# DearCaat/MHIM-MIL

Hardware: AMD Instinct MI355X
Metric: patch-instances/sec through MHIM fwd+bwd, N=10k D=1024 (higher is better)
Workload: dtype f32; 1 GPU; c2: MHIM(ABMIL) train step, one bag N=10000 D=1024 per GPU per step (teacher fwd + select + student fwd + bwd + Adam + EMA); rotating_bags_per_gpu=8, matrix_core_form=bf16x3, parallelism=dp1, launch=hipGraph replay, one graph per resident bag

## Files before the change

include/mhimx.h:

```cpp
#ifndef MHIMX_H
#define MHIMX_H

#include <stdint.h>

#ifdef __cplusplus
extern "C" {
#endif

#define MHIMX_VERSION 620

enum { MHIMX_ACT_NONE = 0, MHIMX_ACT_RELU = 1, MHIMX_ACT_GELU = 2, MHIMX_ACT_TANH = 3 };

enum { MHIMX_PREC_F32 = 0, MHIMX_PREC_F16S = 1, MHIMX_PREC_BF16X3 = 2 };

const char* mhimx_last_error(void);
int mhimx_version(void);


typedef struct {
  const float* A; int64_t lda; const int64_t* rows;
  const float* B; int64_t ldb;
  float* C; int64_t ldc;
  int64_t M, N, K;
  const float* bias;
// ... 206 lines not shown
typedef struct { int64_t H, cell0, ncell, out0, out1; } mhimx_ppeg_band;
int64_t mhimx_ppeg_side(int64_t N, int64_t* wrapN);
int mhimx_ppeg_band_fwd(void* stream, const float* xb, const mhimx_ppeg_band* band, int64_t C, const float* wc, const float* bc, float* y);
int64_t mhimx_ppeg_band_bwd_ws_floats(int64_t n_out, int64_t C);
int mhimx_ppeg_band_bwd(void* stream, const float* dyb, const float* xb, const mhimx_ppeg_band* band, int64_t n_dw, int64_t C, const float* wc,
                        float* dx, float* dwc, float* dbc, float* ws);
int mhimx_scale_heads(void* stream, const float* v, int64_t ldv, const float* a, int64_t lda, int64_t dh, int64_t T, int64_t C, float* out);

int64_t mhimx_select_ws_bytes(int64_t N);
int mhimx_select_mask(void* stream, const float* score, int64_t N, int64_t k, int64_t n_sel, int32_t largest,
                      const int64_t* perm, const int64_t* other, int64_t n_other,
                      int64_t* mask_ids, int64_t* len_keep_dev, int64_t* topk_sorted ,
                      void* ws, int64_t ws_bytes);

int mhimx_select_rows(void* stream, const float* score, int64_t N, int64_t k, int64_t n_sel, int32_t largest,
                      uint64_t rand_seed, const uint64_t* tick, int64_t merge_R, int64_t* rows_out, int64_t* mask_ids,
                      void* ws, int64_t ws_bytes, int32_t merge_first );

int mhimx_select_rows_img(void* stream, const float* score, int64_t N, int64_t k, int64_t n_sel, int32_t largest, uint64_t rand_seed,
                          const uint64_t* tick, int64_t merge_R, int64_t* rows_out, int64_t* rows_img, int64_t img_merge_off, void* ws,
                          int64_t ws_bytes, int32_t merge_first);
int mhimx_vote_scores(void* stream, const float* attn, int64_t H, int64_t N, int64_t k, int32_t largest,
                      float* vote, void* ws, int64_t ws_bytes);

int mhimx_compose_ids(void* stream, const int64_t* a, const int64_t* b, int64_t* out, int64_t n);
int mhimx_random_perm(void* stream, int64_t n, uint64_t seed, const uint64_t* tick, const int64_t* src, int64_t* out);

typedef struct { int64_t row0, N, k, n_sel, merge_R, out0; uint64_t seed; } mhimx_select_bag;
int64_t mhimx_select_rows_many_ws_bytes(int32_t n_bags, const mhimx_select_bag* bags);
int mhimx_select_rows_many(void* stream, const float* score, int32_t n_bags, const mhimx_select_bag* bags, const uint64_t* tick,
                           int64_t* rows_out, void* ws, int64_t ws_bytes, int32_t merge_first);

typedef struct {
  int64_t E; int64_t k;
  int64_t heads; int64_t dim_head;
  const float* q_param;
  const float* ln_w; const float* ln_b;
  const float* wkv; const float* wq; const float* wo; const float* bo;
  const float* wkv_t; const float* wq_t; const float* wo_t;
  float mm;
  float drop_p; uint64_t drop_seed;
  int32_t prec;
  const uint64_t* drop_tick;
  const float* wkv_frag;
  const int64_t* x_rows;
  int32_t prepared;
  int64_t own_lo, own_n;
  float rep;
  int32_t rows_done;
} mhimx_merge;
int64_t mhimx_merge_ws_bytes(int64_t R, int64_t E, int64_t k, int64_t heads, int64_t dim_head);
int mhimx_merge_fwd(void* stream, const mhimx_merge* m, const float* X, int64_t R, float* z, float* q_new,
                    int32_t update_q, void* ws, int64_t ws_bytes);
typedef struct {
  float* d_ln_w; float* d_ln_b; float* d_wkv; float* d_wq; float* d_wo; float* d_bo;
  int32_t accumulate; int32_t splits;
  mhimx_reduce_list* defer;
} mhimx_merge_grad;
int64_t mhimx_merge_part_floats(void);
int mhimx_merge_fwd_part(void* stream, const mhimx_merge* m, const float* X, int64_t R, float* part, void* ws, int64_t ws_bytes);
int mhimx_merge_fwd_finish(void* stream, const mhimx_merge* m, const float* parts, int32_t W, int64_t R, float* z, float* q_new,
                           int32_t update_q, void* ws, int64_t ws_bytes);
int mhimx_merge_bwd(void* stream, const mhimx_merge* m, const float* X, int64_t R, const float* dz, float* dX,
                    const mhimx_merge_grad* g, void* ws, int64_t ws_bytes);
int mhimx_merge_bwd_park(const mhimx_merge* m, const float* X, int64_t R, const float* dz, float* dX, const mhimx_merge_grad* g, void* ws,
                         int64_t ws_bytes);

int mhimx_act_bwd(void* stream, float* dH, const float* H, const float* pre, int64_t M, int64_t E, int32_t act,
                  float drop_p, uint64_t drop_seed, const uint8_t* drop_mask, const int64_t* rows, float* colsum_out,
                  int32_t accumulate, void* ws, int64_t ws_bytes, const uint64_t* drop_tick);
int mhimx_mul_colsum(void* stream, float* dH, const float* dact, int64_t M, int64_t E, float* colsum_out, int32_t accumulate,
                     void* ws, int64_t ws_bytes, mhimx_reduce_list* defer );
int mhimx_rows_dpre(void* stream, const float* dH, const void* dact16, const int64_t* rows, int64_t L, int64_t E, float* dpre,
                    float* colsum_out, int32_t accumulate, void* ws, int64_t ws_bytes, mhimx_reduce_list* defer );
int64_t mhimx_wgrad_image_bytes(int64_t L, int64_t E);
int mhimx_rows_dpre_image(void* stream, const float* dH, const void* dact16, const int64_t* rows, int64_t L, int64_t E, void* img,
                          float* colsum_out, int32_t accumulate, void* ws, int64_t ws_bytes, mhimx_reduce_list* defer );
int mhimx_rows_dpre_image_c(void* stream, const float* dH_compact, const void* dact16, const int64_t* rows, int64_t L, int64_t E, void* img,
                            float* colsum_out, int32_t accumulate, void* ws, int64_t ws_bytes, mhimx_reduce_list* defer );
int mhimx_rows_dpre_image_k(void* stream, const float* dH, const void* dact16, const uint8_t* keep, int64_t N, int64_t E, void* img,
                            float* colsum_out, int32_t accumulate, void* ws, int64_t ws_bytes, mhimx_reduce_list* defer );
typedef struct {
  const void* img;
  const float* X; int64_t ldx; int64_t n_bag_rows;
  const int64_t* rows;
  int64_t L, E, D;
  float* C; int64_t ldc; int32_t accumulate;
  float* ws; int64_t ws_floats;
  mhimx_reduce_list* defer;
  int32_t ride_tail;
  const void* ximg;
} mhimx_bag_wgrad_args;
int64_t mhimx_wgrad_ws_floats(int64_t L, int64_t E, int64_t D);
int mhimx_bag_wgrad(void* stream, const mhimx_bag_wgrad_args* a);
int64_t mhimx_wgrad_multi_ws_floats(int64_t L, int64_t E, int64_t D, int32_t n_bags);
int mhimx_bag_wgrad_multi(void* stream, const mhimx_bag_wgrad_args* bags, int32_t n_bags);
int mhimx_shard_flags(void* stream, const int64_t* rows_all, int64_t R, int64_t Lk, int64_t lo, int64_t n, int64_t k_tokens,
                      int32_t tokens_live, uint8_t* excl);
int mhimx_shard_gather(void* stream, const float* H, int64_t E, const int64_t* rows, int64_t R, int64_t lo, int64_t n, float* out);
int mhimx_shard_scatter(void* stream, const float* dX, int64_t E, const int64_t* rows, int64_t R, int64_t lo, int64_t n, float* dH);
int mhimx_colsum(void* stream, const float* X, int64_t M, int64_t E, float* out, int32_t accumulate,
                 void* ws, int64_t ws_bytes);

int mhimx_head_fwd_bwd(void* stream, const float* z, const float* t, const float* wp, const float* bp,
                       const int64_t* label_dev, int64_t E, int64_t C, float temp_t, float main_alpha,
                       float aux_alpha, float inv_accum, float* logits, float* losses, float* g_z, float* d_wp,
// ... 320 lines not shown
```

mhim_mil_amd/_lib.py:

```python
from __future__ import annotations

import ctypes as C
import os

HERE = os.path.dirname(os.path.abspath(__file__))
LIB_PATH = os.path.join(HERE, os.environ.get("MHIMX_LIB_NAME", "libmhimx.so"))

c_f32p = C.c_void_p
c_i64p = C.c_void_p
c_u8p = C.c_void_p

ABI_VERSION = 620

ACT = {None: 0, "none": 0, "identity": 0, "relu": 1, "gelu": 2, "tanh": 3}
PREC = {"f32": 0, "f16s": 1, "bf16x3": 2}


def act_code(name, allowed):
    n = name.lower() if isinstance(name, str) else None
    return ACT[n] if n in allowed else 0


class GemmNT(C.Structure):
    _fields_ = [("A", c_f32p), ("lda", C.c_int64), ("rows", c_i64p),
# ... 54 lines not shown


class ParkedGemm(C.Structure):
    _fields_ = [("pending", C.c_int32), ("reserved", C.c_int32), ("blob", C.c_ubyte * 128)]


class ReduceListC(C.Structure):
    _fields_ = [("j", ReduceJob * REDUCE_MAX), ("n", C.c_int32), ("side", SideWork), ("parked", ParkedGemm), ("pre", SideWork)]


class GemmTN(C.Structure):
    _fields_ = [("A", c_f32p), ("lda", C.c_int64),
                ("B", c_f32p), ("ldb", C.c_int64), ("rows", c_i64p),
                ("C", c_f32p), ("ldc", C.c_int64),
                ("M", C.c_int64), ("K1", C.c_int64), ("K2", C.c_int64),
                ("splits", C.c_int32), ("ws", c_f32p),
                ("accumulate", C.c_int32), ("prec", C.c_int32), ("ws_floats", C.c_int64),
                ("defer", C.c_void_p)]


class Scorer(C.Structure):
    _fields_ = [("E", C.c_int64), ("A", C.c_int64), ("act", C.c_int32), ("gated", C.c_int32), ("prec", C.c_int32),
                ("wa", c_f32p), ("ba", c_f32p), ("wb", c_f32p), ("bb", c_f32p), ("wc", c_f32p), ("bc", c_f32p),
                ("wa_frag", c_f32p), ("gate_drop_p", C.c_float), ("gate_drop_seed", C.c_uint64)]


class PoolIO(C.Structure):
    _fields_ = [("T1", c_f32p), ("M1", C.c_int64), ("T2", c_f32p), ("M2", C.c_int64),
                ("s", c_f32p), ("stats", c_f32p), ("z", c_f32p), ("u_pre", c_f32p),
                ("wp", c_f32p), ("C", C.c_int64), ("cproj", c_f32p),
                ("ws", C.c_void_p), ("ws_bytes", C.c_int64), ("bp", c_f32p), ("pscore", c_f32p), ("rows1", c_i64p),
                ("excl", C.c_void_p), ("ride_jobs", C.c_void_p), ("n_ride_jobs", C.c_int32),
                ("phase", C.c_int32), ("tail_tokens", C.c_int32), ("ride_merge", C.c_void_p), ("ride_X", c_f32p), ("ride_R", C.c_int64),
                ("ride_ws", C.c_void_p), ("ride_ws_bytes", C.c_int64), ("rode_merge", C.c_int32), ("tail_wa_t", c_f32p), ("tail_row0", C.c_int64),
                ("no_backward", C.c_int32)]


class PoolGrad(C.Structure):
    _fields_ = [("g_z", c_f32p), ("dT1", c_f32p), ("dT2", c_f32p),
                ("d_wa", c_f32p), ("d_ba", c_f32p), ("d_wb", c_f32p), ("d_bb", c_f32p), ("d_wc", c_f32p),
                ("d_bc", c_f32p), ("wa_t", c_f32p), ("wb_t", c_f32p),
                ("accumulate", C.c_int32), ("splits", C.c_int32), ("defer", C.c_void_p), ("wa_t_frag", c_f32p),
                ("img", C.c_void_p), ("img_dact", C.c_void_p), ("img_part", c_f32p), ("img_rows", C.c_int64)]


class Merge(C.Structure):
    _fields_ = [("E", C.c_int64), ("k", C.c_int64), ("heads", C.c_int64), ("dim_head", C.c_int64),
                ("q_param", c_f32p), ("ln_w", c_f32p), ("ln_b", c_f32p),
                ("wkv", c_f32p), ("wq", c_f32p), ("wo", c_f32p), ("bo", c_f32p),
                ("wkv_t", c_f32p), ("wq_t", c_f32p), ("wo_t", c_f32p),
                ("mm", C.c_float), ("drop_p", C.c_float), ("drop_seed", C.c_uint64), ("prec", C.c_int32), ("drop_tick", C.c_void_p),
                ("wkv_frag", c_f32p), ("x_rows", c_i64p), ("prepared", C.c_int32), ("own_lo", C.c_int64), ("own_n", C.c_int64),
                ("rep", C.c_float), ("rows_done", C.c_int32)]


class MergeGrad(C.Structure):
    _fields_ = [("d_ln_w", c_f32p), ("d_ln_b", c_f32p), ("d_wkv", c_f32p), ("d_wq", c_f32p), ("d_wo", c_f32p),
                ("d_bo", c_f32p), ("accumulate", C.c_int32), ("splits", C.c_int32), ("defer", C.c_void_p)]


_P = C.c_void_p
_I64 = C.c_int64
_I32 = C.c_int32
_F = C.c_float
_U64 = C.c_uint64


class Nys(C.Structure):
    _fields_ = [("q", C.c_void_p), ("k", C.c_void_p), ("v", C.c_void_p), ("ld", C.c_int64), ("T", C.c_int64),
                ("ql", C.c_void_p), ("kl", C.c_void_p), ("ldl", C.c_int64), ("scale", C.c_float),
                ("ws", C.c_void_p), ("ws_floats", C.c_int64)]


class BmmStep(C.Structure):
    _fields_ = [("A", C.c_void_p), ("B", C.c_void_p), ("C", C.c_void_p), ("PN", C.c_void_p), ("PT", C.c_void_p),
                ("PN2", C.c_void_p), ("PT2", C.c_void_p), ("D", C.c_void_p), ("D2", C.c_void_p), ("alpha", C.c_float), ("ident", C.c_float),
                ("alpha2", C.c_float), ("ident2", C.c_float), ("dscale", C.c_float), ("d2scale", C.c_float), ("kind", C.c_int32)]


class OptimArgs(C.Structure):
    _fields_ = [("p", C.c_void_p), ("g", C.c_void_p), ("m", C.c_void_p), ("v", C.c_void_p), ("teacher", C.c_void_p),
                ("n_train", C.c_int64), ("n_all", C.c_int64), ("step", C.c_int64), ("step_dev", C.c_void_p),
                ("lr", C.c_float), ("lr_table", C.c_void_p), ("lr_len", C.c_int64),
                ("beta1", C.c_float), ("beta2", C.c_float), ("eps", C.c_float), ("weight_decay", C.c_float), ("grad_scale", C.c_float),
                ("ema_mm", C.c_float), ("mm_table", C.c_void_p), ("mm_len", C.c_int64), ("zero_grad", C.c_int32),
                ("g_extra", C.c_void_p), ("n_extra", C.c_int64), ("extra_pitch", C.c_int64), ("clip_norm", C.c_float),
                ("ws", C.c_void_p), ("ws_floats", C.c_int64), ("fold", C.c_void_p), ("extra_lo", C.c_int64), ("extra_only", C.c_int32)]


class StepParams(C.Structure):
    _fields_ = [(n, C.c_void_p) for n in ("w1", "b1", "wa", "wc", "wp", "bp", "q", "ln_w", "ln_b", "wkv", "wq", "wo", "bo")]


class StepGrads(C.Structure):
    _fields_ = [(n, C.c_void_p) for n in ("w1", "b1", "wa", "wc", "wp", "bp", "ln_w", "ln_b", "wkv", "wq", "wo", "bo")]


class StepCfg(C.Structure):
    _fields_ = [("D", C.c_int64), ("E", C.c_int64), ("A", C.c_int64), ("C", C.c_int64), ("k", C.c_int64),
                ("act", C.c_int32), ("da_act", C.c_int32), ("attn2score", C.c_int32),
                ("drop_p_teacher", C.c_float), ("drop_p_student", C.c_float), ("merge_drop_p", C.c_float), ("merge_mm", C.c_float),
                ("temp_t", C.c_float), ("main_alpha", C.c_float), ("aux_alpha", C.c_float),
                ("student", StepParams), ("teacher", StepParams), ("grad", StepGrads),
                ("p", C.c_void_p), ("g", C.c_void_p), ("m", C.c_void_p), ("v", C.c_void_p), ("p_teacher", C.c_void_p),
                ("n_train", C.c_int64), ("n_all", C.c_int64),
                ("lr", C.c_float), ("beta1", C.c_float), ("beta2", C.c_float), ("eps", C.c_float), ("weight_decay", C.c_float), ("ema_mm", C.c_float),
# ... 128 lines not shown
                                        "H_teacher", "H_student", "dact", "score", "rows_all", "tokens")] + [
        ("row0", C.c_int64 * DSMIL_MHIM_WINDOW_MAX), ("tok0", C.c_int64 * DSMIL_MHIM_WINDOW_MAX)]


RAGGED_WINDOW_MAX = 32
RAGGED_WINDOW_MAX_ROWS = 524288


class RaggedWindowBag(C.Structure):
    _fields_ = [("X", c_f32p), ("ldx", C.c_int64), ("N", C.c_int64), ("label_dev", C.c_void_p), ("cnt", StepCounts), ("seeds", StepSeeds)]


class RaggedWindowLayout(C.Structure):
    _fields_ = [(n, C.c_int64) for n in ("total", "rows", "logits", "losses", "score", "rows_all", "H_teacher", "H_student", "dact", "dpre",
                                        "z_teacher", "z_student")] + [("row0", C.c_int64 * RAGGED_WINDOW_MAX)]


class SurvSpec(C.Structure):
    _fields_ = [("alpha", C.c_float), ("eps", C.c_float), ("censor_dev", C.c_void_p * INFER_MAX), ("risk", C.c_void_p)]


SYMBOLS = {
    "mhimx_last_error": (C.c_char_p, []),
    "mhimx_version": (C.c_int, []),
    "mhimx_gemm_nt": (C.c_int, [_P, C.POINTER(GemmNT)]),
    "mhimx_pool_finalize": (C.c_int, [_P, _P, _P, _P, _I64, _I64, _P, _P, _P, _P, _P, _I64, _I64, _P]),
    "mhimx_proj_score_parts": (_I64, [_I64]),
    "mhimx_proj_score_xch_floats": (_I64, [_I64]),
    "mhimx_bag_project": (C.c_int, [_P, C.POINTER(BagProject)]),
    "mhimx_bag_project_multi": (C.c_int, [_P, _P, _I32]),
    "mhimx_gemm_nn": (C.c_int, [_P, C.POINTER(GemmNT), _F, _I32, _P]),
    "mhimx_prep_batch": (C.c_int, [_P, C.POINTER(PrepJob), _I32]),
    "mhimx_pair_planes": (C.c_int, [_P, _P, _I64, _I64, _I64, _P]),
    "mhimx_lse_merge": (C.c_int, [_P, _P, _I64, _I64, _P, _P]),
    "mhimx_gemm_batched": (C.c_int, [_P, _I32, C.POINTER(GemmNT), _I32, _I64, _I64, _I64, _F, _I32, _P]),
    "mhimx_gemm_tn": (C.c_int, [_P, C.POINTER(GemmTN)]),
    "mhimx_transpose": (C.c_int, [_P, _P, _P, _I64, _I64]),
    "mhimx_abmil_pool_ws_bytes": (_I64, [_I64, _I64, _I64, _I32]),
    "mhimx_abmil_pool_fwd": (C.c_int, [_P, C.POINTER(Scorer), C.POINTER(PoolIO)]),
    "mhimx_abmil_pool_bwd": (C.c_int, [_P, C.POINTER(Scorer), C.POINTER(PoolIO), C.POINTER(PoolGrad)]),
    "mhimx_softmax_from_stats": (C.c_int, [_P, _P, _P, _P, _I64]),
    "mhimx_pseudo_score": (C.c_int, [_P, _P, _P, _P, _P, _P, _P, _I64, _I64]),
    "mhimx_select_ws_bytes": (_I64, [_I64]),
    "mhimx_select_mask": (C.c_int, [_P, _P, _I64, _I64, _I64, _I32, _P, _P, _I64, _P, _P, _P, _P, _I64]),
    "mhimx_select_rows": (C.c_int, [_P, _P, _I64, _I64, _I64, _I32, _U64, _P, _I64, _P, _P, _P, _I64, _I32]),
    "mhimx_select_rows_img": (C.c_int, [_P, _P, _I64, _I64, _I64, _I32, _U64, _P, _I64, _P, _P, _I64, _P, _I64, _I32]),
    "mhimx_vote_scores": (C.c_int, [_P, _P, _I64, _I64, _I64, _I32, _P, _P, _I64]),
    "mhimx_compose_ids": (C.c_int, [_P, _P, _P, _P, _I64]),
    "mhimx_random_perm": (C.c_int, [_P, _I64, _U64, _P, _P, _P]),
    "mhimx_select_rows_many_ws_bytes": (_I64, [_I32, _P]),
    "mhimx_select_rows_many": (C.c_int, [_P, _P, _I32, _P, _P, _P, _P, _I64, _I32]),
    "mhimx_merge_ws_bytes": (_I64, [_I64, _I64, _I64, _I64, _I64]),
    "mhimx_merge_fwd": (C.c_int, [_P, C.POINTER(Merge), _P, _I64, _P, _P, _I32, _P, _I64]),
    "mhimx_merge_part_floats": (_I64, []),
    "mhimx_merge_fwd_part": (C.c_int, [_P, C.POINTER(Merge), _P, _I64, _P, _P, _I64]),
    "mhimx_merge_fwd_finish": (C.c_int, [_P, C.POINTER(Merge), _P, _I32, _I64, _P, _P, _I32, _P, _I64]),
    "mhimx_merge_bwd": (C.c_int, [_P, C.POINTER(Merge), _P, _I64, _P, _P, C.POINTER(MergeGrad), _P, _I64]),
    "mhimx_merge_bwd_park": (C.c_int, [C.POINTER(Merge), _P, _I64, _P, _P, C.POINTER(MergeGrad), _P, _I64]),
    "mhimx_act_bwd": (C.c_int, [_P, _P, _P, _P, _I64, _I64, _I32, _F, _U64, _P, _P, _P, _I32, _P, _I64, _P]),
    "mhimx_softmax_cols": (C.c_int, [_P, _P, _P, _I64, _I64, _F]),
    "mhimx_softmax_cols_bwd": (C.c_int, [_P, _P, _P, _P, _I64, _I64, _F]),
    "mhimx_colmax": (C.c_int, [_P, _P, _I64, _I64, _P, _P]),
    "mhimx_rowmax": (C.c_int, [_P, _P, _I64, _I64, _P]),
    "mhimx_dsmil_head": (C.c_int, [_P, _P, _P, _P, _P, _P, _I64, _I64, _F, _F, _F, _F, _P, _P, _P, _P, _P]),
    "mhimx_mul_colsum": (C.c_int, [_P, _P, _P, _I64, _I64, _P, _I32, _P, _I64, _P]),
    "mhimx_rows_dpre": (C.c_int, [_P, _P, _P, _P, _I64, _I64, _P, _P, _I32, _P, _I64, _P]),
    "mhimx_bmm_affine": (C.c_int, [_P, _I32, _P, _I32, _I64, _I64, _I64, C.c_float, C.c_float]),
    "mhimx_bmm_affine2": (C.c_int, [_P, _I32, _P, _I32, _I64, _I64, _I64, C.c_float, C.c_float, _P, C.c_float, C.c_float]),
    "mhimx_bmm_affine_pair": (C.c_int, [_P, _I32, C.POINTER(GemmNT), _F, _F, _I32, C.POINTER(GemmNT), _F, _F, _I32, _I64]),
    "mhimx_shard_flags": (C.c_int, [_P, _P, _I64, _I64, _I64, _I64, _I64, _I32, _P]),
    "mhimx_shard_gather": (C.c_int, [_P, _P, _I64, _P, _I64, _I64, _I64, _P]),
    "mhimx_shard_scatter": (C.c_int, [_P, _P, _I64, _P, _I64, _I64, _I64, _P]),
    "mhimx_rows_dpre_image": (C.c_int, [_P, _P, _P, _P, _I64, _I64, _P, _P, _I32, _P, _I64, _P]),
    "mhimx_rows_dpre_image_c": (C.c_int, [_P, _P, _P, _P, _I64, _I64, _P, _P, _I32, _P, _I64, _P]),
    "mhimx_rows_dpre_image_k": (C.c_int, [_P, _P, _P, _P, _I64, _I64, _P, _P, _I32, _P, _I64, _P]),
    "mhimx_wgrad_image_bytes": (_I64, [_I64, _I64]),
    "mhimx_wgrad_ws_floats": (_I64, [_I64, _I64, _I64]),
    "mhimx_bag_wgrad": (C.c_int, [_P, _P]),
    "mhimx_bag_wgrad_multi": (C.c_int, [_P, _P, _I32]),
    "mhimx_wgrad_multi_ws_floats": (C.c_int64, [_I64, _I64, _I64, _I32]),
    "mhimx_reduce_flush": (C.c_int, [_P, _P]),
    "mhimx_cls_metrics_ws_bytes": (C.c_int64, [_I64, _I64, _I64]),
    "mhimx_cls_metrics": (C.c_int, [_P, _P, _I64, _P, _I64, _I64, _I32, _P, _I64, _P, _P, _I64]),
    "mhimx_surv_nll": (C.c_int, [_P, _P, _I64, _P, _P, _I64, _I64, _F, _F, _F, _P, _P, _P]),
    "mhimx_cindex_ws_bytes": (C.c_int64, [_I64, _I64]),
    "mhimx_cindex": (C.c_int, [_P, _P, _P, _P, _I64, _P, _I64, _F, _P, _P, _I64]),
    "mhimx_colsum": (C.c_int, [_P, _P, _I64, _I64, _P, _I32, _P, _I64]),
    "mhimx_head_fwd_bwd": (C.c_int, [_P, _P, _P, _P, _P, _P, _I64, _I64, _F, _F, _F, _F, _P, _P, _P, _P, _P, _I32, _P, _P]),
    "mhimx_head_surv_fwd_bwd": (C.c_int, [_P, _P, _P, _P, _P, _P, _P, _I64, _I64, _F, _F, _F, _F, _F, _F, _P, _P, _P, _P, _P, _P, _I32]),
    "mhimx_adam_ema": (C.c_int, [_P, _P, _P, _P, _P, _P, _I64, _I64, _I64, _F, _F, _F, _F, _F, _F, _F, _I32, _P, _P, _I64]),
    "mhimx_bmm_chain": (C.c_int, [_P, C.POINTER(BmmStep), _I32, _I32, _P]),
    "mhimx_optim_step": (C.c_int, [_P, C.POINTER(OptimArgs)]),
    "mhimx_stream_copy": (C.c_int, [_P, _P, _P, _I64]),
    "mhimx_tick": (C.c_int, [_P, _P]),
    "mhimx_layernorm_fwd": (C.c_int, [_P, _P, _I64, _I64, _P, _P, _P, _P, _P]),
    "mhimx_layernorm_bwd": (C.c_int, [_P, _P, _P, _I64, _I64, _P, _P, _P, _P, _P, _P, _I32, _P]),
    "mhimx_layernorm_bwd_res": (C.c_int, [_P, _P, _P, _I64, _I64, _P, _P, _P, _P, _P, _P, _P, _I32, _P]),
    "mhimx_dropout_apply": (C.c_int, [_P, _P, _P, _I64, _I64, _F, _U64, _P]),
    "mhimx_dropout_apply_proj": (C.c_int, [_P, _P, _P, _I64, _I64, _F, _U64, _P]),
    "mhimx_softmax_rows": (C.c_int, [_P, _P, _P, _I64, _I64, _F]),
    "mhimx_softmax_rows_bwd": (C.c_int, [_P, _P, _P, _P, _I64, _I64, _F]),
    "mhimx_landmark_mean": (C.c_int, [_P, _P, _I64, _I64, _I64, _I64, _P]),
    "mhimx_landmark_mean_bwd": (C.c_int, [_P, _P, _I64, _I64, _I64, _P, _I64, _I32]),
    "mhimx_affine_ident": (C.c_int, [_P, _P, _P, _I64, _I64, _F, _F]),
    "mhimx_axpby": (C.c_int, [_P, _P, _P, _I64, _F, _F]),
    "mhimx_pinv_init": (C.c_int, [_P, _P, _I64, _I64, _P, _P, _P]),
# ... 92 lines not shown
```

mhim_mil_amd/csrc/common.hpp:

```cpp
#pragma once
#include <hip/hip_runtime.h>
#include <stdint.h>
#include <stdio.h>
#include <string>
#include <type_traits>

#include "../../include/mhimx.h"

namespace mhimx {

void set_error(const std::string& s);
int fail(int code, const char* fmt, ...);
const std::string& last_error();

#define MHIMX_CHECK_ARG(cond, ...)                      \
  do {                                                  \
    if (!(cond)) return ::mhimx::fail(-1, __VA_ARGS__); \
  } while (0)

#define MHIMX_HIP(expr)                                                                      \
  do {                                                                                       \
    hipError_t _e = (expr);                                                                  \
    if (_e != hipSuccess) return ::mhimx::fail((int)_e, "%s: %s", #expr, hipGetErrorString(_e)); \
  } while (0)
// ... 38 lines not shown
}
inline bool reduce_slabs_as_parts(int64_t splits, int64_t K1, int64_t K2, int64_t ldo) { return splits >= 32 && ldo == K2 && K1 * K2 <= 16384; }
inline mhimx_reduce_job reduce_job_slabs(const float* ws, int64_t splits, int64_t K1, int64_t K2, int64_t ldo, float* out, int accumulate) {
  if (reduce_slabs_as_parts(splits, K1, K2, ldo)) return reduce_job_parts(ws, splits, K1 * K2, K1 * K2, out, accumulate);
  mhimx_reduce_job j = {};
  j.kind = 1; j.accumulate = accumulate; j.parts = ws; j.out = out; j.G = splits; j.K1 = K1; j.K2 = K2; j.ldo = ldo;
  return j;
}

int reduce_parts_now(hipStream_t st, const float* part, int64_t G, int64_t W, int64_t ld, float* out, int accumulate);
int reduce_slabs_now(hipStream_t st, const float* ws, float* C, int64_t K1, int64_t K2, int64_t ldc, int splits, int accumulate,
                     int batch = 1, int64_t sC = 0);

inline mhimx_optim_args optim_args_of(const mhimx_step_cfg& c, int64_t host_step, bool with_teacher) {
  mhimx_optim_args o = {};
  o.p = c.p; o.g = c.g; o.m = c.m; o.v = c.v; o.n_train = c.n_train; o.n_all = c.n_all; o.step = host_step; o.step_dev = c.opt_step;
  o.lr = c.lr; o.lr_table = c.lr_table; o.lr_len = c.lr_len; o.beta1 = c.beta1; o.beta2 = c.beta2; o.eps = c.eps; o.weight_decay = c.weight_decay;
  o.grad_scale = 1.f; o.zero_grad = 1;
  if (with_teacher) { o.teacher = c.p_teacher; o.ema_mm = c.ema_mm; o.mm_table = c.mm_table; o.mm_len = c.mm_len; }
  return o;
}

inline int prep_counters(const mhimx_step_cfg& c, mhimx_prep_job* j) {
  int n = 0;
  j[n++] = mhimx_prep_job{3, nullptr, reinterpret_cast<float*>(c.tick), 1, 1};
  if (c.opt_step) j[n++] = mhimx_prep_job{3, nullptr, reinterpret_cast<float*>(c.opt_step), 1, 1};
  return n;
}

struct Arena {
  char* base;
  int64_t cap, off;
  Arena(void* p, int64_t bytes) : base((char*)p), cap(bytes), off(0) {}
  template <typename T>
  T* take(int64_t n) {
    int64_t b = align_up(n * (int64_t)sizeof(T), 256);
    T* r = (T*)(base + off);
    off += b;
    return r;
  }
  bool ok() const { return off <= cap && (base != nullptr || off == 0); }
};

constexpr int BAG_BATCH_MAX = MHIMX_WINDOW_MAX;
struct BagBatch {
  int32_t n, pad;
  uint64_t lo[3], span[3];
  int64_t stride[3];
  uint64_t dsel[BAG_BATCH_MAX], dmca[BAG_BATCH_MAX];
  uint64_t tab_key, tab[BAG_BATCH_MAX];
};
const BagBatch& cur_batch();
void set_batch(const BagBatch* b);
inline dim3 bgrid(unsigned x, unsigned y = 1) { return dim3(x, y, cur_batch().n > 0 ? (unsigned)cur_batch().n : 1u); }

#define MHIMX_DEV __device__ __forceinline__

template <typename T>
MHIMX_DEV T* bag_ptr(T* p, const BagBatch& bb) {
  const unsigned bag = blockIdx.z;
  if (bag == 0) return p;
  const uint64_t a = reinterpret_cast<uint64_t>(p);
#pragma unroll
  for (int r = 0; r < 3; ++r)
    if (a - bb.lo[r] < bb.span[r]) return reinterpret_cast<T*>(a + (uint64_t)bag * (uint64_t)bb.stride[r]);
  if (a == bb.tab_key) return reinterpret_cast<T*>(bb.tab[bag]);
  return p;
}
#define MHIMX_BAG(p) p = ::mhimx::bag_ptr(p, bb)
MHIMX_DEV uint64_t bag_sel_seed(uint64_t s, const BagBatch& bb) { return blockIdx.z ? s + bb.dsel[blockIdx.z] : s; }
MHIMX_DEV uint64_t bag_mca_seed(uint64_t s, const BagBatch& bb) { return blockIdx.z ? s + bb.dmca[blockIdx.z] : s; }

MHIMX_DEV float erf_fast(float x) {
  const float ax = fabsf(x);
  const float t = __frcp_rn(fmaf(0.3275911f, ax, 1.f));
  float p = fmaf(1.061405429f, t, -1.453152027f);
  p = fmaf(p, t, 1.421413741f);
  p = fmaf(p, t, -0.284496736f);
  p = fmaf(p, t, 0.254829592f);
  const float r = 1.f - p * t * __expf(-ax * ax);
  return copysignf(r, x);
}

MHIMX_DEV float tanh_fast(float x) {
  const float t = __expf(-2.f * fabsf(x));
  return copysignf((1.f - t) * __frcp_rn(1.f + t), x);
}

MHIMX_DEV float act_fwd(float x, int act) {
  switch (act) {
    case MHIMX_ACT_RELU: return x > 0.f ? x : 0.f;
    case MHIMX_ACT_GELU: return 0.5f * x * (1.f + erf_fast(x * 0.70710678118654752440f));
    case MHIMX_ACT_TANH: return tanh_fast(x);
    default: return x;
  }
}

MHIMX_DEV float act_grad(float x, float y, int act) {
  switch (act) {
    case MHIMX_ACT_RELU: return y > 0.f ? 1.f : 0.f;
    case MHIMX_ACT_GELU: {
      const float phi = 0.39894228040143267794f * __expf(-0.5f * x * x);
      return 0.5f * (1.f + erf_fast(x * 0.70710678118654752440f)) + x * phi;
    }
    case MHIMX_ACT_TANH: return 1.f - y * y;
    default: return 1.f;
// ... 114 lines not shown
```

mhim_mil_amd/csrc/dsmil_mhim.hip:

```cpp
#include <math.h>
#include <string.h>

#include "infer_tab.hpp"

namespace mhimx {

bool merge2_ok(const mhimx_merge* m, int64_t R);
int64_t merge2_ws_bytes(int64_t R, int64_t k);

namespace {

constexpr int DM_Q = 128, DM_MAXC = 16, DM_ROWS = RG_ROWS, DM_T = 256;
constexpr int DM_MAX = MHIMX_DSMIL_MHIM_WINDOW_MAX;
constexpr int DM_GATHER_Y = 64;
static_assert(DM_MAX == MHIMX_INFER_MAX, "the by-value bag table is the inference call's");

typedef _Float16 dm_h4 __attribute__((ext_vector_type(4)));

struct DmCnt {
  int64_t tok0[DM_MAX], mrg0[DM_MAX];
  int32_t len_keep[DM_MAX], Lk[DM_MAX], tslot[DM_MAX];
};
struct DmLabels { const int64_t* p[DM_MAX]; };

__global__ __launch_bounds__(DM_T) void dm_gather_kernel(InferTab tab, DmCnt cn, const float* __restrict__ Hs, const int64_t* __restrict__ rows_all,
                                                         int k, float* __restrict__ T, float* __restrict__ Xm, int32_t* __restrict__ pos) {
  const int bag = blockIdx.x;
  int64_t N = tab.N[0], orow0 = tab.row0[0], tok0 = cn.tok0[0], mrg0 = cn.mrg0[0];
  int len_keep = cn.len_keep[0], Lk = cn.Lk[0], tslot = cn.tslot[0];
  RG_PICK(N, tab.N, bag) RG_PICK(orow0, tab.row0, bag) RG_PICK(tok0, cn.tok0, bag) RG_PICK(mrg0, cn.mrg0, bag)
  RG_PICK(len_keep, cn.len_keep, bag) RG_PICK(Lk, cn.Lk, bag) RG_PICK(tslot, cn.tslot, bag)
  const int tid = threadIdx.x, lane = tid & 63, wave = tid >> 6;
  const int64_t* rows = rows_all + orow0;
  const f32x4 z4 = f32x4{0.f, 0.f, 0.f, 0.f};
  for (int j = blockIdx.y * (DM_T / 64) + wave; j < len_keep; j += (DM_T / 64) * gridDim.y) {
    const int64_t r = rows[j];
    const bool ok = r >= 0 && r < N;
    const f32x4* src = reinterpret_cast<const f32x4*>(Hs + (orow0 + (ok ? r : 0)) * IE);
    f32x4* dst = reinterpret_cast<f32x4*>(j < Lk ? T + (tok0 + j) * IE : Xm + (mrg0 + (j - Lk)) * IE);
    f32x4 v0 = src[lane], v1 = src[lane + 64];
    if (!ok) { v0 = z4; v1 = z4; }
    dst[lane] = v0;
    dst[lane + 64] = v1;
    if (ok && lane == 0) pos[orow0 + r] = j;
  }
  if (blockIdx.y == 0) {
    const int first = Lk + k;
    f32x4* dst = reinterpret_cast<f32x4*>(T + (tok0 + first) * IE);
    for (int f = tid; f < (tslot - first) * (IE / 4); f += DM_T) dst[f] = z4;
  }
}

MHIMX_DEV float dm_blk_max(float v, float* red) {
  const int lane = threadIdx.x & 63, wave = threadIdx.x >> 6;
  v = wave_max(v);
  if (lane == 0) red[wave] = v;
  __syncthreads();
  float r = red[0];
#pragma unroll
  for (int w = 1; w < 8; ++w) r = fmaxf(r, red[w]);
  __syncthreads();
// ... 142 lines not shown
}

__global__ __launch_bounds__(DM_T) void dm_scatter_kernel(InferTab tab, DmCnt cn, const int64_t* __restrict__ rows_all, const int32_t* __restrict__ pos,
                                                          const float* __restrict__ dT, const float* __restrict__ dXm,
                                                          const _Float16* __restrict__ dact, float* __restrict__ dpre, float* __restrict__ part) {
  __shared__ f32x4 half[IE / 4];
  __shared__ int64_t srow[DM_ROWS];
  const int tile = blockIdx.x, tid = threadIdx.x;
  const int64_t r0 = (int64_t)tile * DM_ROWS;
  RG_FIND_BAG(r0, row0)
  int64_t N = tab.N[0], orow0 = tab.row0[0], tok0 = cn.tok0[0], mrg0 = cn.mrg0[0];
  int len_keep = cn.len_keep[0], Lk = cn.Lk[0];
  RG_PICK(N, tab.N, bag) RG_PICK(orow0, tab.row0, bag) RG_PICK(tok0, cn.tok0, bag) RG_PICK(mrg0, cn.mrg0, bag)
  RG_PICK(len_keep, cn.len_keep, bag) RG_PICK(Lk, cn.Lk, bag)
  if (tid < DM_ROWS) {
    const int64_t rin = r0 - orow0 + tid;
    int64_t s = -1;
    if (rin < N) {
      const int p = pos[r0 + tid];
      if (p >= 0 && p < len_keep && rows_all[orow0 + p] == rin) s = p < Lk ? tok0 + p : -2 - (mrg0 + (p - Lk));
    }
    srow[tid] = s;
  }
  __syncthreads();
  const int c4 = tid & 127, par = tid >> 7;
  f32x4 sum = f32x4{0.f, 0.f, 0.f, 0.f};
#pragma unroll 4
  for (int i = 0; i < DM_ROWS / 2; ++i) {
    const int r = 2 * i + par;
    const int64_t s = srow[r];
    f32x4 d = f32x4{0.f, 0.f, 0.f, 0.f};
    if (s != -1) {
      const float* src = s >= 0 ? dT + s * IE : dXm + (-2 - s) * IE;
      const f32x4 g = reinterpret_cast<const f32x4*>(src)[c4];
      const dm_h4 a = *(reinterpret_cast<const dm_h4*>(dact + (r0 + r) * IE) + c4);
#pragma unroll
      for (int q = 0; q < 4; ++q) d[q] = g[q] * (float)a[q];
    }
    *(reinterpret_cast<f32x4*>(dpre + (r0 + r) * IE) + c4) = d;
#pragma unroll
    for (int q = 0; q < 4; ++q) sum[q] += d[q];
  }
  if (par == 1) half[c4] = sum;
  __syncthreads();
  if (par == 0) {
    const f32x4 o = half[c4];
#pragma unroll
    for (int q = 0; q < 4; ++q) sum[q] += o[q];
    *(reinterpret_cast<f32x4*>(part + (int64_t)tile * IE) + c4) = sum;
  }
}

struct DmLay {
  int64_t w1p_t, w1p_s, vp_t, q0f_t, q2f_t, vp, vtp, q0f, q2f, q2tf, q0tf, wo_t;
  int64_t logits, losses, logits_bag, logits_ins, B, crit, B_t, lb_t, lg_t, li_t, crit_t, qmax_t, qmax, stats, gli, dB, delta, dqmax, dwfcc_part,
      dbfcc_part, dwi_part, dbi_part;
  int64_t H_t, H_s, dact, V_t, Q_t, cls_t, score, rows_all, pos, db1_part, pmax_t, parg_t, pm_t, pl_t, pB_t, slab_1;
  int64_t T, V, dhv, Q, cls, da, U1, dPQ, dP1, pmax, parg, pm, pl, pB, dbv_part, dbq0_part, dbq2_part, dqm_part, slab_v, slab_q0, slab_q2;
  int64_t Xm, dXm, merge_ws[DM_MAX], merge_ws_bytes[DM_MAX], sel_ws, sel_ws_bytes, sel_perm, sel_ids, sel_rows, sel_lk;
  int64_t total, rows, trows, mrows;
  int32_t steps, tsteps, s1, s1_per, sv, sv_per, sq0, sq0_per, sq2, sq2_per;
};

mhimx_merge dm_merge_params(const mhimx_dsmil_mhim_cfg& c) {
  mhimx_merge m = {};
  m.E = c.base.E; m.k = c.k; m.heads = 8; m.dim_head = 64;
  m.q_param = c.q; m.ln_w = c.merge.ln_w; m.ln_b = c.merge.ln_b; m.wkv = c.merge.wkv; m.wq = c.merge.wq; m.wo = c.merge.wo; m.bo = c.merge.bo;
  m.mm = c.merge_mm; m.prec = MHIMX_PREC_BF16X3; m.drop_tick = c.base.tick; m.rep = 1.f; m.drop_p = c.merge_drop_p;
  return m;
}

bool dm_params_ok(const mhimx_dsmil_params& p) {
  return p.w1 && p.b1 && p.wi && p.bi && p.wq0 && p.bq0 && p.wq2 && p.bq2 && p.wv && p.bv && p.wfcc && p.bfcc;
}
bool dm_params_aligned(const mhimx_dsmil_params& p) {
  return aligned16(p.w1) && aligned16(p.b1) && aligned16(p.wi) && aligned16(p.wq0) && aligned16(p.wq2) && aligned16(p.wv) && aligned16(p.bv);
}

int check_dm(const mhimx_dsmil_mhim_cfg* cfg, int32_t n_bags, const mhimx_ragged_window_bag* bags, int32_t xdt = MHIMX_X_F32) {
  const char* who = "dsmil_mhim_window";
  if (int r = rg_check_xdt(who, xdt)) return r;
  MHIMX_CHECK_ARG(cfg && bags, "dsmil_mhim_window: null configuration / bag list");
  MHIMX_CHECK_ARG(n_bags >= 1 && n_bags <= DM_MAX, "dsmil_mhim_window: 1..%d bags per window (got %d)", DM_MAX, n_bags);
  const mhimx_dsmil_train_cfg* c = &cfg->base;
  MHIMX_CHECK_ARG(c->E == IE && c->C >= 1 && c->C <= DM_MAXC && c->D > 0 && c->D % 256 == 0 && c->D <= (1 << 20),
                  "dsmil_mhim_window: shapes outside the ragged MHIM(DSMIL) window (E = 512, q width 128, 1 <= C <= %d, D %% 256 == 0, D <= 2^20)", DM_MAXC);
  MHIMX_CHECK_ARG(cfg->k >= 1 && 8 * cfg->k <= 48, "dsmil_mhim_window: merge_k outside 1..6 (8 k <= 48)");
  MHIMX_CHECK_ARG(c->act >= MHIMX_ACT_NONE && c->act <= MHIMX_ACT_TANH, "dsmil_mhim_window: unknown activation");
  MHIMX_CHECK_ARG(c->drop_p >= 0.f && c->drop_p < 1.f && cfg->drop_p_teacher >= 0.f && cfg->drop_p_teacher < 1.f && cfg->merge_drop_p >= 0.f &&
                      cfg->merge_drop_p < 1.f,
                  "dsmil_mhim_window: dropout probability outside [0,1)");
  MHIMX_CHECK_ARG(cfg->temp_t > 0.f, "dsmil_mhim_window: the distillation temperature must be positive");
  MHIMX_CHECK_ARG(dm_params_ok(c->param), "dsmil_mhim_window: null student parameter");
  MHIMX_CHECK_ARG(dm_params_ok(cfg->teacher), "dsmil_mhim_window: null teacher parameter");
  MHIMX_CHECK_ARG(dm_params_aligned(c->param) && dm_params_aligned(cfg->teacher),
                  "dsmil_mhim_window: the feature, i_classifier, q and v weights of both models must be 16-byte aligned");
  const mhimx_dsmil_grads& g = c->grad;
  MHIMX_CHECK_ARG(g.w1 && g.b1 && g.wi && g.bi && g.wq0 && g.bq0 && g.wq2 && g.bq2 && g.wv && g.bv && g.wfcc && g.bfcc,
                  "dsmil_mhim_window: null gradient view");
  const mhimx_dsmil_merge_params& m = cfg->merge;
  MHIMX_CHECK_ARG(m.ln_w && m.ln_b && m.wkv && m.wq && m.wo && m.bo && cfg->q, "dsmil_mhim_window: null Merge parameter / global queries");
  MHIMX_CHECK_ARG(aligned16(m.ln_w) && aligned16(m.ln_b) && aligned16(m.wkv) && aligned16(m.wq) && aligned16(m.wo) && aligned16(cfg->q) &&
                      (!cfg->q_out || aligned16(cfg->q_out)),
                  "dsmil_mhim_window: the Merge weights and the global queries must be 16-byte aligned");
  const mhimx_dsmil_merge_grads& mg = cfg->merge_grad;
  MHIMX_CHECK_ARG(mg.ln_w && mg.ln_b && mg.wkv && mg.wq && mg.wo && mg.bo, "dsmil_mhim_window: null Merge gradient view");
  MHIMX_CHECK_ARG(c->tick, "dsmil_mhim_window: the device dropout / draw counter (tick) is required");
// ... 11 lines not shown
    MHIMX_CHECK_ARG(merge2_ok(&mw, n.R), "dsmil_mhim_window: bag %d: the Merge entry points' projection-free form does not take R = %lld", b,
                    (long long)n.R);
    rows += align_up(q.N, DM_ROWS);
    MHIMX_CHECK_ARG(rows <= MHIMX_DSMIL_MHIM_WINDOW_MAX_ROWS, "dsmil_mhim_window: bag %d: %lld rows in the window's bag space up to this bag, at most %d", b,
                    (long long)rows, MHIMX_DSMIL_MHIM_WINDOW_MAX_ROWS);
  }
  return 0;
}

void dm_layout(const mhimx_dsmil_mhim_cfg* cfg, int32_t n_bags, const mhimx_ragged_window_bag* bags, DmLay* w, InferTab* tab, InferTab* tab2, DmCnt* cn,
               int64_t* row0_out, int64_t* tok0_out) {
  const int64_t E = cfg->base.E, D = cfg->base.D, C = cfg->base.C, k = cfg->k, n = n_bags;
  RgCount cnt, cnt2;
  int64_t mrows = 0, sel_b = 0, perm_n = 0, ids_n = 0, rows_n = 0;
  for (int b = 0; b < n_bags; ++b) {
    const mhimx_ragged_window_bag& q = bags[b];
    const int64_t M = q.cnt.Lk + k, tslot = align_up(M, DM_ROWS);
    if (row0_out) row0_out[b] = cnt.rows;
    if (tok0_out) tok0_out[b] = cnt2.rows;
    if (cn) {
      cn->tok0[b] = cnt2.rows; cn->mrg0[b] = mrows; cn->len_keep[b] = (int32_t)q.cnt.len_keep; cn->Lk[b] = (int32_t)q.cnt.Lk;
      cn->tslot[b] = (int32_t)tslot;
    }
    rg_tab_add(tab, cnt, b, q.X, q.ldx, q.N, align_up(q.N, DM_ROWS));
    rg_tab_add(tab2, cnt2, b, nullptr, IE, M, tslot);
    mrows += q.cnt.R;
    auto up = [](int64_t& a, int64_t v) { if (v > a) a = v; };
    up(sel_b, mhimx_select_ws_bytes(q.N));
    if (q.N > 16384) { up(perm_n, q.cnt.k_top); up(ids_n, q.N); up(rows_n, q.cnt.len_keep); }
  }
  rg_tab_close(tab, cnt, n_bags);
  rg_tab_close(tab2, cnt2, n_bags);
  const int64_t rows = cnt.rows, parts = cnt.parts, trows = cnt2.rows, tparts = cnt2.parts;
  w->rows = rows; w->trows = trows; w->mrows = mrows;
  w->steps = (int32_t)(rows / DM_ROWS);
  w->tsteps = (int32_t)(trows / DM_ROWS);
  const int s1_room = pw_split_k(w->steps, 8, 8, &w->s1, &w->s1_per);
  const int sv_room = pw_split_k(w->tsteps, 16, 4, &w->sv, &w->sv_per);
  const int sq0_room = pw_split_k(w->tsteps, 64, 4, &w->sq0, &w->sq0_per);
  const int sq2_room = pw_split_k(w->tsteps, 64, 2, &w->sq2, &w->sq2_per);
  Arena ar(nullptr, 0);
  w->w1p_t = ar.off; ar.take<float>(E * D);
  w->w1p_s = ar.off; ar.take<float>(E * D);
  w->vp_t = ar.off; ar.take<float>(E * E);
  w->q0f_t = ar.off; ar.take<float>(DM_Q * E);
  w->q2f_t = ar.off; ar.take<float>(DM_Q * DM_Q);
  w->vp = ar.off; ar.take<float>(E * E);
  w->vtp = ar.off; ar.take<float>(E * E);
  w->q0f = ar.off; ar.take<float>(DM_Q * E);
  w->q2f = ar.off; ar.take<float>(DM_Q * DM_Q);
  w->q2tf = ar.off; ar.take<float>(DM_Q * DM_Q);
  w->q0tf = ar.off; ar.take<float>(DM_Q * E);
  w->wo_t = ar.off; ar.take<float>(512 * E);
  w->logits = ar.off; ar.take<float>(n * C);
  w->losses = ar.off; ar.take<float>(n * 3);
  w->logits_bag = ar.off; ar.take<float>(n * C);
  w->logits_ins = ar.off; ar.take<float>(n * C);
  w->B = ar.off; ar.take<float>(n * C * E);
  w->crit = ar.off; ar.take<int64_t>(n * C);
  w->B_t = ar.off; ar.take<float>(n * C * E);
  w->lb_t = ar.off; ar.take<float>(n * C);
  w->lg_t = ar.off; ar.take<float>(n * C);
  w->li_t = ar.off; ar.take<float>(n * C);
  w->crit_t = ar.off; ar.take<int64_t>(n * C);
  w->qmax_t = ar.off; ar.take<float>(n * DM_MAXC * DM_Q);
  w->qmax = ar.off; ar.take<float>(n * DM_MAXC * DM_Q);
  w->stats = ar.off; ar.take<float>(n * DM_MAXC * 2);
  w->gli = ar.off; ar.take<float>(n * DM_MAXC);
  w->dB = ar.off; ar.take<float>(n * DM_MAXC * E);
  w->delta = ar.off; ar.take<float>(n * DM_MAXC);
  w->dqmax = ar.off; ar.take<float>(n * DM_MAXC * DM_Q);
  w->dwfcc_part = ar.off; ar.take<float>(n * C * C * E);
  w->dbfcc_part = ar.off; ar.take<float>(n * C);
  w->dwi_part = ar.off; ar.take<float>(n * C * E);
  w->dbi_part = ar.off; ar.take<float>(n * C);
  w->H_t = ar.off; ar.take<float>(rows * E);
  w->H_s = ar.off; ar.take<float>(rows * E);
  w->dact = ar.off; ar.take<_Float16>(rows * E);
  w->V_t = ar.off; ar.take<float>(rows * E);
  w->Q_t = ar.off; ar.take<float>(rows * DM_Q);
  w->cls_t = ar.off; ar.take<float>(rows * DM_MAXC);
  w->score = ar.off; ar.take<float>(rows);
  w->rows_all = ar.off; ar.take<int64_t>(rows);
  w->pos = ar.off; ar.take<int32_t>(rows);
  w->db1_part = ar.off; ar.take<float>((int64_t)w->steps * E);
  w->pmax_t = ar.off; ar.take<float>(parts * DM_MAXC);
  w->parg_t = ar.off; ar.take<int32_t>(parts * DM_MAXC);
  w->pm_t = ar.off; ar.take<float>(parts * DM_MAXC);
  w->pl_t = ar.off; ar.take<float>(parts * DM_MAXC);
  w->pB_t = ar.off; ar.take<float>(parts * C * E);
  w->slab_1 = ar.off; ar.take<float>((int64_t)s1_room * E * D);
  w->T = ar.off; ar.take<float>(trows * E);
  w->V = ar.off; ar.take<float>(trows * E);
  w->dhv = ar.off; ar.take<float>(trows * E);
  w->Q = ar.off; ar.take<float>(trows * DM_Q);
  w->cls = ar.off; ar.take<float>(trows * DM_MAXC);
  w->da = ar.off; ar.take<float>(trows * DM_MAXC);
  w->U1 = ar.off; ar.take<float>(trows * DM_Q);
  w->dPQ = ar.off; ar.take<float>(trows * DM_Q);
  w->dP1 = ar.off; ar.take<float>(trows * DM_Q);
  w->pmax = ar.off; ar.take<float>(tparts * DM_MAXC);
  w->parg = ar.off; ar.take<int32_t>(tparts * DM_MAXC);
  w->pm = ar.off; ar.take<float>(tparts * DM_MAXC);
  w->pl = ar.off; ar.take<float>(tparts * DM_MAXC);
  w->pB = ar.off; ar.take<float>(tparts * C * E);
  w->dbv_part = ar.off; ar.take<float>((int64_t)w->tsteps * E);
  w->dbq0_part = ar.off; ar.take<float>((int64_t)w->tsteps * DM_Q);
  w->dbq2_part = ar.off; ar.take<float>((int64_t)w->tsteps * DM_Q);
  w->dqm_part = ar.off; ar.take<float>((int64_t)w->tsteps * DM_MAXC * DM_Q);
  w->slab_v = ar.off; ar.take<float>((int64_t)sv_room * E * E);
  w->slab_q0 = ar.off; ar.take<float>((int64_t)sq0_room * DM_Q * E);
  w->slab_q2 = ar.off; ar.take<float>((int64_t)sq2_room * DM_Q * DM_Q);
  w->Xm = ar.off; ar.take<float>(mrows * E);
  w->dXm = ar.off; ar.take<float>(mrows * E);
  for (int b = 0; b < n_bags; ++b) {
    w->merge_ws_bytes[b] = merge2_ws_bytes(bags[b].cnt.R, k);
    w->merge_ws[b] = ar.off; ar.take<char>(w->merge_ws_bytes[b]);
  }
  w->sel_ws_bytes = sel_b; w->sel_ws = ar.off; ar.take<char>(sel_b);
  w->sel_perm = ar.off; ar.take<int64_t>(perm_n);
  w->sel_ids = ar.off; ar.take<int64_t>(ids_n);
  w->sel_rows = ar.off; ar.take<int64_t>(rows_n);
  w->sel_lk = ar.off; ar.take<int64_t>(1);
  w->total = ar.off;
}

}

}

using namespace mhimx;

extern "C" int mhimx_dsmil_mhim_window_layout_of(const mhimx_dsmil_mhim_cfg* cfg, int32_t n_bags, const mhimx_ragged_window_bag* bags,
                                                 mhimx_dsmil_mhim_window_layout* out) {
  MHIMX_CHECK_ARG(out, "dsmil_mhim_window_layout: null output");
  if (int r = check_dm(cfg, n_bags, bags)) return r;
  DmLay w;
  memset(out, 0, sizeof(*out));
  dm_layout(cfg, n_bags, bags, &w, nullptr, nullptr, nullptr, out->row0, out->tok0);
  out->total = w.total; out->rows = w.rows; out->tok_rows = w.trows; out->logits = w.logits; out->losses = w.losses; out->logits_bag = w.logits_bag;
  out->logits_ins = w.logits_ins; out->B = w.B; out->crit = w.crit; out->B_teacher = w.B_t; out->H_teacher = w.H_t; out->H_student = w.H_s;
  out->dact = w.dact; out->score = w.score; out->rows_all = w.rows_all; out->tokens = w.T;
  return 0;
}

extern "C" int64_t mhimx_dsmil_mhim_window_ws_bytes(const mhimx_dsmil_mhim_cfg* cfg, int32_t n_bags, const mhimx_ragged_window_bag* bags) {
  if (int r = check_dm(cfg, n_bags, bags)) return r;
  DmLay w;
  dm_layout(cfg, n_bags, bags, &w, nullptr, nullptr, nullptr, nullptr, nullptr);
  return w.total;
}

extern "C" int mhimx_dsmil_mhim_window_run(void* stream, const mhimx_dsmil_mhim_cfg* cfg, int32_t n_bags, const mhimx_ragged_window_bag* bags,
                                           int64_t host_step, void* ws, int64_t ws_bytes, int32_t update, int32_t x_dtype) {
  if (int r = check_dm(cfg, n_bags, bags, x_dtype)) return r;
  for (int b = 0; b < n_bags; ++b) {
    MHIMX_CHECK_ARG(bags[b].X && aligned16(bags[b].X), "dsmil_mhim_window: bag %d: null or unaligned rows", b);
    MHIMX_CHECK_ARG(bags[b].label_dev, "dsmil_mhim_window: bag %d: null label", b);
  }
  const mhimx_dsmil_train_cfg& c = cfg->base;
  MHIMX_CHECK_ARG(!update || (c.p && c.g && c.m && c.v && c.n_train > 0 && c.n_all >= c.n_train), "dsmil_mhim_window: update needs the flat optimiser buffers");
  DmLay w;
  InferTab tab = {}, tab2 = {};
  DmCnt cn = {};
  dm_layout(cfg, n_bags, bags, &w, &tab, &tab2, &cn, nullptr, nullptr);
  tab.pad = x_dtype;
  tab2.pad = MHIMX_X_F32;
  if (int r = rg_check_ws("dsmil_mhim_window", ws, ws_bytes, w.total)) return r;
  const mhimx_dsmil_params &P = c.param, &Tp = cfg->teacher;
  hipStream_t st = (hipStream_t)stream;
  char* base = static_cast<char*>(ws);
  auto F = [&](int64_t off) { return reinterpret_cast<float*>(base + off); };
  const int D = (int)c.D, C = (int)c.C;
  const int64_t k = cfg->k;
  float *H_t = F(w.H_t), *H_s = F(w.H_s), *V_t = F(w.V_t), *Q_t = F(w.Q_t), *score = F(w.score);
  float *T = F(w.T), *V = F(w.V), *dhv = F(w.dhv), *Q = F(w.Q), *Xm = F(w.Xm), *dXm = F(w.dXm);
  float* dpre = V_t;
  _Float16* dact = reinterpret_cast<_Float16*>(base + w.dact);
  int64_t* rows_space = reinterpret_cast<int64_t*>(base + w.rows_all);
  int32_t* pos = reinterpret_cast<int32_t*>(base + w.pos);
  int64_t* crit = reinterpret_cast<int64_t*>(base + w.crit);
  const uint64_t* tick = c.tick;
  float* q_dst = cfg->q_out ? cfg->q_out : cfg->q;

  mhimx_merge mw_prep = dm_merge_params(*cfg);
  {
    mhimx_prep_job jobs[24];
    int n = 0;
    jobs[n++] = mhimx_prep_job{3, nullptr, reinterpret_cast<float*>(c.tick), 1, 1};
    if (c.opt_step) jobs[n++] = mhimx_prep_job{3, nullptr, reinterpret_cast<float*>(c.opt_step), 1, 1};
    jobs[n++] = mhimx_prep_job{1, Tp.w1, F(w.w1p_t), c.E, c.D};
    jobs[n++] = mhimx_prep_job{1, P.w1, F(w.w1p_s), c.E, c.D};
    jobs[n++] = mhimx_prep_job{1, Tp.wv, F(w.vp_t), c.E, c.E};
    jobs[n++] = mhimx_prep_job{4, Tp.wq0, F(w.q0f_t), DM_Q, c.E};
    jobs[n++] = mhimx_prep_job{4, Tp.wq2, F(w.q2f_t), DM_Q, DM_Q};
    jobs[n++] = mhimx_prep_job{1, P.wv, F(w.vp), c.E, c.E};
    jobs[n++] = mhimx_prep_job{7, P.wv, F(w.vtp), c.E, c.E};
    jobs[n++] = mhimx_prep_job{4, P.wq0, F(w.q0f), DM_Q, c.E};
    jobs[n++] = mhimx_prep_job{4, P.wq2, F(w.q2f), DM_Q, DM_Q};
    jobs[n++] = mhimx_prep_job{5, P.wq2, F(w.q2tf), DM_Q, DM_Q};
    jobs[n++] = mhimx_prep_job{5, P.wq0, F(w.q0tf), DM_Q, c.E};
    jobs[n++] = mhimx_prep_job{0, cfg->merge.wo, F(w.wo_t), c.E, 512};
    if (cfg->q_out) jobs[n++] = mhimx_prep_job{2, cfg->q, cfg->q_out, 1, k * c.E};
    for (int b = 0; b < n_bags && b < 8; ++b)
      jobs[n++] = mhimx_prep_job{6, reinterpret_cast<const float*>(&mw_prep), reinterpret_cast<float*>(base + w.merge_ws[b]), bags[b].cnt.R, w.merge_ws_bytes[b]};
    if (int r = mhimx_prep_batch(stream, jobs, n)) return r;
  }
  {
    PureWinDrop dr = {};
    dr.tick = tick; dr.dact = dact;
    for (int b = 0; b < n_bags; ++b) dr.seed[b] = bags[b].seeds.drop_teacher;
    dr.drop_p = cfg->drop_p_teacher;
    if (int r = pure_window_project(st, tab, dr, D, F(w.w1p_t), Tp.b1, c.act, H_t)) return r;
    for (int b = 0; b < n_bags; ++b) dr.seed[b] = bags[b].seeds.drop_student;
    dr.drop_p = c.drop_p;
    if (int r = pure_window_project(st, tab, dr, D, F(w.w1p_s), P.b1, c.act, H_s)) return r;
  }
  InferTab tabv = tab;
  for (int b = 0; b < n_bags; ++b) { tabv.X[b] = H_t + tab.row0[b] * IE; tabv.ldx[b] = IE; }
  tabv.pad = MHIMX_X_F32;
  if (int r = infer_project(st, tabv, IE, F(w.vp_t), Tp.bv, MHIMX_ACT_RELU, V_t)) return r;
  if (int r = dsmil_rows_crit_pool(st, tab, H_t, V_t, F(w.q0f_t), Tp.bq0, F(w.q2f_t), Tp.bq2, Tp.wi, Tp.bi, C, Q_t, F(w.cls_t), F(w.pmax_t),
                                   reinterpret_cast<int32_t*>(base + w.parg_t), F(w.qmax_t), F(w.li_t), reinterpret_cast<int64_t*>(base + w.crit_t),
                                   F(w.pm_t), F(w.pl_t), F(w.pB_t), cfg->cls_attn ? score : nullptr))
    return r;
  if (int r = dsmil_finalize(st, tab, F(w.pm_t), F(w.pl_t), F(w.pB_t), Q_t, F(w.qmax_t), Tp.wfcc, Tp.bfcc, C, F(w.li_t), F(w.lb_t), F(w.lg_t), F(w.B_t),
                             cfg->cls_attn ? nullptr : score))
    return r;
  {
    mhimx_select_bag sb[DM_MAX];
    for (int b = 0; b < n_bags; ++b) {
      const mhimx_step_counts& n = bags[b].cnt;
      sb[b] = mhimx_select_bag{tab.row0[b], bags[b].N, n.k_top, n.n_sel, n.R, tab.row0[b], bags[b].seeds.select};
    }
    SelLargeWs lw;
    lw.perm = reinterpret_cast<int64_t*>(base + w.sel_perm); lw.ids = reinterpret_cast<int64_t*>(base + w.sel_ids);
    lw.rows = reinterpret_cast<int64_t*>(base + w.sel_rows); lw.lk = reinterpret_cast<int64_t*>(base + w.sel_lk);
    lw.sel_ws = base + w.sel_ws; lw.sel_ws_bytes = w.sel_ws_bytes;
    if (int r = select_bags_check("dsmil_mhim_window", n_bags, sb)) return r;
    if (int r = select_rows_many_launch(st, score, n_bags, sb, tick, rows_space, lw, 0)) return r;
  }
  hipLaunchKernelGGL(dm_gather_kernel, dim3((unsigned)n_bags, DM_GATHER_Y), dim3(DM_T), 0, st, tab, cn, H_s, rows_space, (int)k, T, Xm, pos);
  MHIMX_LAUNCH_CHECK();

  for (int b = 0; b < n_bags; ++b) {
    if (b >= 8 && b % 8 == 0) {
      mhimx_prep_job jobs[8];
      int n = 0;
      for (int q = b; q < n_bags && q < b + 8; ++q)
        jobs[n++] = mhimx_prep_job{6, reinterpret_cast<const float*>(&mw_prep), reinterpret_cast<float*>(base + w.merge_ws[q]), bags[q].cnt.R, w.merge_ws_bytes[q]};
      if (int r = mhimx_prep_batch(stream, jobs, n)) return r;
    }
    mhimx_merge mw = mw_prep;
    mw.drop_seed = bags[b].seeds.mca; mw.prepared = 1;
    if (int r = mhimx_merge_fwd(stream, &mw, Xm + cn.mrg0[b] * IE, bags[b].cnt.R, T + (cn.tok0[b] + cn.Lk[b]) * IE, nullptr, 0, base + w.merge_ws[b],
                                w.merge_ws_bytes[b]))
      return r;
  }

  InferTab tabt = tab2;
  for (int b = 0; b < n_bags; ++b) tabt.X[b] = T + tab2.row0[b] * IE;
  if (int r = infer_project(st, tabt, IE, F(w.vp), P.bv, MHIMX_ACT_RELU, V)) return r;
  if (int r = dsmil_rows_crit_pool(st, tab2, T, V, F(w.q0f), P.bq0, F(w.q2f), P.bq2, P.wi, P.bi, C, Q, F(w.cls), F(w.pmax),
                                   reinterpret_cast<int32_t*>(base + w.parg), F(w.qmax), F(w.logits_ins), crit, F(w.pm), F(w.pl), F(w.pB)))
    return r;
  {
    DmLabels lab = {};
    for (int b = 0; b < n_bags; ++b) lab.p[b] = bags[b].label_dev;
    const float* Bt = cfg->aux_alpha != 0.f ? F(w.B_t) : nullptr;
    hipLaunchKernelGGL(dm_head_kernel, dim3((unsigned)n_bags), dim3(RG_FIN_T), 0, st, tab2, lab, F(w.pm), F(w.pl), F(w.pB), T, P.wfcc, P.bfcc, F(w.logits_ins),
                       crit, Bt, C, cfg->temp_t, c.main_alpha, cfg->aux_alpha, 1.f / (float)n_bags, F(w.logits_bag), F(w.logits), F(w.losses), F(w.B),
                       F(w.stats), F(w.gli), F(w.dB), F(w.delta), F(w.dwfcc_part), F(w.dbfcc_part), F(w.dwi_part), F(w.dbi_part));
    MHIMX_LAUNCH_CHECK();
  }
  if (int r = dw_rows1(st, tab2, w.tsteps, V, Q, F(w.qmax), F(w.stats), F(w.dB), F(w.delta), C, F(w.da), F(w.dbv_part), F(w.dqm_part))) return r;
  for (int b = 0; b < n_bags; ++b) tabt.X[b] = V + tab2.row0[b] * IE;
  if (int r = infer_project(st, tabt, IE, F(w.vtp), nullptr, MHIMX_ACT_NONE, dhv)) return r;
  if (int r = dw_dqmax(st, tab2, F(w.dqm_part), F(w.dqmax))) return r;
  if (int r = dw_rows2_plain(st, tab2, w.tsteps, T, Q, F(w.da), F(w.qmax), F(w.dqmax), crit, F(w.gli), P.wi, F(w.q0f), P.bq0, F(w.q2tf), F(w.q0tf), C, dhv,
                             F(w.U1), F(w.dPQ), F(w.dP1), F(w.dbq0_part), F(w.dbq2_part)))
    return r;
  if (int r = pw_wgrad_rows(st, tab2, V, IE, IE, T, IE, IE, w.tsteps, w.sv, w.sv_per, F(w.slab_v))) return r;
  if (int r = pw_wgrad_rows(st, tab2, F(w.dPQ), DM_Q, DM_Q, F(w.U1), DM_Q, DM_Q, w.tsteps, w.sq2, w.sq2_per, F(w.slab_q2))) return r;
  if (int r = pw_wgrad_rows(st, tab2, F(w.dP1), DM_Q, DM_Q, T, IE, IE, w.tsteps, w.sq0, w.sq0_per, F(w.slab_q0))) return r;

  for (int b = 0; b < n_bags; ++b) {
    mhimx_merge mwb = mw_prep;
    mwb.drop_seed = bags[b].seeds.mca; mwb.wo_t = F(w.wo_t); mwb.prepared = 0;
    mhimx_reduce_list lst;
    memset(&lst, 0, sizeof(lst));
    mhimx_merge_grad mg = {};
    const mhimx_dsmil_merge_grads& G_ = cfg->merge_grad;
    mg.d_ln_w = G_.ln_w; mg.d_ln_b = G_.ln_b; mg.d_wkv = G_.wkv; mg.d_wq = G_.wq; mg.d_wo = G_.wo; mg.d_bo = G_.bo;
    mg.accumulate = b > 0 ? 1 : 0; mg.splits = 8; mg.defer = &lst;
    if (int r = mhimx_merge_bwd(stream, &mwb, Xm + cn.mrg0[b] * IE, bags[b].cnt.R, dhv + (cn.tok0[b] + cn.Lk[b]) * IE, dXm + cn.mrg0[b] * IE, &mg,
                                base + w.merge_ws[b], w.merge_ws_bytes[b]))
      return r;
    if (int r = mhimx_reduce_flush(stream, &lst)) return r;
  }

  hipLaunchKernelGGL(dm_scatter_kernel, dim3((unsigned)w.steps), dim3(DM_T), 0, st, tab, cn, rows_space, pos, dhv, dXm, dact, dpre, F(w.db1_part));
  MHIMX_LAUNCH_CHECK();
  if (int r = pw_wgrad_bagx(st, tab, dpre, D, w.steps, w.s1, w.s1_per, F(w.slab_1))) return r;
// ... 27 lines not shown
```

mhim_mil_amd/csrc/errors.hip:

```cpp
#include <stdarg.h>

#include "common.hpp"

namespace mhimx {
static thread_local std::string g_err;
void set_error(const std::string& s) { g_err = s; }
int fail(int code, const char* fmt, ...) {
  char buf[512];
  va_list ap;
  va_start(ap, fmt);
  vsnprintf(buf, sizeof(buf), fmt, ap);
  va_end(ap);
  g_err = buf;
  return code;
}
const std::string& last_error() { return g_err; }

static thread_local BagBatch g_batch = {};
const BagBatch& cur_batch() { return g_batch; }
void set_batch(const BagBatch* b) {
  if (b) g_batch = *b;
  else g_batch = BagBatch{};
}
}

extern "C" const char* mhimx_last_error(void) { return mhimx::last_error().c_str(); }
extern "C" int mhimx_version(void) { return MHIMX_VERSION; }
```

mhim_mil_amd/csrc/gemm_dma.hip:

```cpp
#include <string.h>

#include "common.hpp"
#include "mca2_rows.hpp"
#include "prep_jobs.hpp"

namespace mhimx {

typedef float f32x16 __attribute__((ext_vector_type(16)));
typedef float f4 __attribute__((ext_vector_type(4)));
typedef _Float16 h8 __attribute__((ext_vector_type(8)));
typedef __bf16 b8 __attribute__((ext_vector_type(8)));
typedef __attribute__((address_space(1))) const void* gptr_t;
typedef __attribute__((address_space(3))) void* lptr_t;

constexpr int DBM = 128, DBN = 128, DBK = 32, DTHREADS = 256;
constexpr int TILE_BYTES = 128 * DBK * 4;
constexpr int STAGE_BYTES = 2 * TILE_BYTES;
#ifndef MHIMX_NT_STAGES
#define MHIMX_NT_STAGES 2
#endif
constexpr int NSTAGE = MHIMX_NT_STAGES;
constexpr int NT_LDS_BYTES = NSTAGE * STAGE_BYTES > DBM * (DBN + 8) * 4 ? NSTAGE * STAGE_BYTES : DBM * (DBN + 8) * 4;
#define LDS_READ8(x, a, off)                                                                                         \
  asm volatile("ds_read_b128 %0, %8\n\tds_read_b128 %1, %9\n\tds_read_b128 %2, %10\n\tds_read_b128 %3, %11\n\t"       \
// ... 421 lines not shown
        const int64_t i = i0 + wm * 64 + mt * 32 + (e & 3) + 8 * (e >> 2) + 4 * rh;
        float v = acc[mt][nt][e];
        float* p = out + i * ldo + j;
        if (accum) v += *p;
        *p = v;
      }
    }
}


__global__ void pair_planes_kernel(const float* __restrict__ x, int64_t ldx, int64_t M, int64_t K8, float* __restrict__ out) {
  const int64_t n = M * K8;
  for (int64_t i = (int64_t)blockIdx.x * blockDim.x + threadIdx.x; i < n; i += (int64_t)gridDim.x * blockDim.x) {
    const int64_t m = i / K8, g8 = i % K8;
    const f4 a = *reinterpret_cast<const f4*>(x + m * ldx + g8 * 8);
    const f4 b = *reinterpret_cast<const f4*>(x + m * ldx + g8 * 8 + 4);
    b8 hi, lo;
    Frag<MHIMX_PREC_BF16X3>::split2(a, b, hi, lo);
    f4* o = reinterpret_cast<f4*>(out + (m * K8 + g8) * 8);
    o[0] = __builtin_bit_cast(f4, hi);
    o[1] = __builtin_bit_cast(f4, lo);
  }
}
int pair_planes(hipStream_t st, const float* x, int64_t ldx, int64_t M, int64_t K, float* out) {
  MHIMX_CHECK_ARG(x && out && M > 0 && K > 0 && K % 8 == 0 && ldx % 4 == 0 && aligned16(x) && aligned16(out),
                  "pair_planes: K must be a multiple of 8, rows 16-byte aligned");
  const int64_t n = M * (K / 8);
  int64_t blocks = cdiv(n, 256);
  if (blocks > 8192) blocks = 8192;
  hipLaunchKernelGGL(pair_planes_kernel, dim3((unsigned)blocks), dim3(256), 0, st, x, ldx, M, K / 8, out);
  MHIMX_LAUNCH_CHECK();
  return 0;
}

__global__ __launch_bounds__(256) void prep_batch_kernel(PrepJobs pj) {
  __shared__ __attribute__((aligned(16))) float lds[PREP_LDS_FLOATS];
  prep_job_block(pj, (int)blockIdx.x, lds);
}
int merge2_prep_args(const mhimx_merge* m, int64_t R, void* ws, int64_t ws_bytes, Merge2PrepArgs* out);
int prep_jobs_fill(const mhimx_prep_job* jobs, int n, PrepJobs* out) {
  MHIMX_CHECK_ARG(jobs && n >= 1 && n <= MHIMX_PREP_MAX, "prep_batch: 1..%d jobs", MHIMX_PREP_MAX);
  PrepJobs& pj = *out;
  pj.n = n;
  int n_merge = 0;
  for (int i = 0; i < n; ++i) {
    pj.j[i] = jobs[i];
    MHIMX_CHECK_ARG(jobs[i].out && (jobs[i].kind == 3 || jobs[i].kind == 10 || jobs[i].in), "prep_batch: null pointer in job %d", i);
    MHIMX_CHECK_ARG(jobs[i].kind >= 0 && jobs[i].kind <= 10, "prep_batch: unknown job kind");
    if (jobs[i].kind == 6) {
      MHIMX_CHECK_ARG(n_merge < PREP_MERGE_MAX, "prep_batch: at most %d Merge preparation jobs per launch", PREP_MERGE_MAX);
      Merge2PrepArgs m2;
      if (int r = merge2_prep_args(reinterpret_cast<const mhimx_merge*>(jobs[i].in), jobs[i].R, jobs[i].out, jobs[i].C, &m2)) return r;
      if (n_merge == 0) pj.m2 = m2;
      MHIMX_CHECK_ARG(m2.q_param == pj.m2.q_param && m2.wq == pj.m2.wq && m2.wkv == pj.m2.wkv && m2.ln_w == pj.m2.ln_w && m2.k == pj.m2.k,
                      "prep_batch: the Merge preparation jobs of one launch share their parameters");
      MHIMX_CHECK_ARG((m2.w.gq - pj.m2.w.gq) == (m2.w.gtf_aq - pj.m2.w.gtf_aq), "prep_batch: Merge workspace layouts differ");
      pj.m2_shift[n_merge] = m2.w.gq - pj.m2.w.gq;
      pj.j[i].R = n_merge++;
    }
    MHIMX_CHECK_ARG(jobs[i].kind != 5 || (jobs[i].C % 32 == 0 && jobs[i].R % 16 == 0 && aligned16(jobs[i].out)),
                    "prep_batch: the transposed fragment image needs C % 32 == 0, R % 16 == 0 and a 16-byte aligned output");
    MHIMX_CHECK_ARG(jobs[i].kind != 4 || (jobs[i].R % 32 == 0 && jobs[i].C % 16 == 0 && aligned16(jobs[i].in) && aligned16(jobs[i].out)),
                    "prep_batch: the fragment image needs R % 32 == 0, C % 16 == 0 and 16-byte aligned buffers");
    MHIMX_CHECK_ARG(jobs[i].kind != 8 || (jobs[i].C % 32 == 0 && aligned16(jobs[i].in) && aligned16(jobs[i].out)),
                    "prep_batch: the 16-row fragment image needs C % 32 == 0 and 16-byte aligned buffers");
    MHIMX_CHECK_ARG(jobs[i].kind != 9 || (jobs[i].C % 256 == 0 && jobs[i].R >= 1 && aligned16(jobs[i].in) && aligned16(jobs[i].out)),
                    "prep_batch: the bag image needs C % 256 == 0 and 16-byte aligned buffers");
    MHIMX_CHECK_ARG(jobs[i].kind != 7 || (jobs[i].R % 8 == 0 && aligned16(jobs[i].out)), "prep_batch: pairing the transpose needs R % 8 == 0 and a 16-byte aligned output");
    MHIMX_CHECK_ARG(jobs[i].kind != 1 || (jobs[i].C % 8 == 0 && aligned16(jobs[i].in) && aligned16(jobs[i].out)),
                    "prep_batch: pairing needs C % 8 == 0 and 16-byte aligned buffers");
  }
  int first = 0;
  for (int i = 0; i < n; ++i) {
    const int64_t items = (jobs[i].kind == 3 || jobs[i].kind == 10) ? 1 : (jobs[i].kind == 0 ? cdiv(jobs[i].R, 32) * cdiv(jobs[i].C, 32) :
                          (jobs[i].kind == 8 ? cdiv(jobs[i].R, 16) * 16 * jobs[i].C / 8 : jobs[i].R * jobs[i].C / 8));
    int64_t want = jobs[i].kind == 0 ? items : cdiv(items, 256);
    if (jobs[i].kind == 6) want = 64;
    if (jobs[i].kind == 9) want = cdiv(jobs[i].R, 32) * (jobs[i].C / 256);
    if (want < 1) want = 1;
    if (want > 4096) want = 4096;
    pj.first[i] = first;
    first += (int)want;
  }
  pj.first[n] = first;
  return first;
}
int prep_batch(hipStream_t st, const mhimx_prep_job* jobs, int n) {
  PrepJobs pj;
  const int blocks = prep_jobs_fill(jobs, n, &pj);
  if (blocks < 0) return blocks;
  hipLaunchKernelGGL(prep_batch_kernel, dim3((unsigned)blocks), dim3(256), 0, st, pj);
  MHIMX_LAUNCH_CHECK();
  return 0;
}

bool nt_dma_ok(const mhimx_gemm_nt_args& g) {
  return (g.prec == MHIMX_PREC_BF16X3 || g.prec == MHIMX_PREC_F16S) && g.K % DBK == 0 && g.lda % 4 == 0 && g.ldb % 4 == 0 &&
         aligned16(g.A) && aligned16(g.B) && g.M > 16;
}

#ifndef MHIMX_NT_WAVES
#define MHIMX_NT_WAVES 8
#endif
int gemm_nt_dma(hipStream_t st, const mhimx_gemm_nt_args& g) {
  constexpr int NW = MHIMX_NT_WAVES;
  dim3 grid((unsigned)(8 * cdiv(g.N, DBN) * cdiv(cdiv(g.M, DBM), 8)));
  int ksteps = 0, ksplit = 1;
  {
    const int64_t tiles = cdiv(g.N, DBN) * cdiv(g.M, DBM), nk = g.K / DBK;
    const bool plain = !g.bias && !g.rowv && !g.pre && g.act == 0 && g.drop_p == 0.f && !g.drop_mask;
    if (plain && g.ws && tiles <= 128 && nk >= 8) {
      int64_t want = 256 / tiles;
      if (want > nk / 4) want = nk / 4;
      if (want > g.ws_floats / (g.M * g.N)) want = g.ws_floats / (g.M * g.N);
      if (want >= 2) {
        ksteps = (int)cdiv(nk, want);
        ksplit = (int)cdiv(nk, ksteps);
        grid.y = (unsigned)ksplit;
      }
    }
  }
  struct Reduce {
    hipStream_t st; const mhimx_gemm_nt_args& g; int ksplit;
    int run() const {
      if (ksplit <= 1) return 0;
      return reduce_slabs_now(st, g.ws, g.C, g.M, g.N, g.ldc, ksplit, g.accumulate);
    }
  } reduce{st, g, ksplit};
    MHIMX_ONCE_PER_DEVICE(MHIMX_HIP(hipFuncSetAttribute((const void*)gemm_nt_dma_kernel<MHIMX_PREC_BF16X3, NW>, hipFuncAttributeMaxDynamicSharedMemorySize, NT_LDS_BYTES)); MHIMX_HIP(hipFuncSetAttribute((const void*)gemm_nt_dma_kernel<MHIMX_PREC_F16S, NW>, hipFuncAttributeMaxDynamicSharedMemorySize, NT_LDS_BYTES)));
  if (g.paired) {
// ... 86 lines not shown
```

mhim_mil_amd/csrc/mca.hip:

```cpp
#include <math.h>

#include "common.hpp"

namespace mhimx {

int gemm_nt(hipStream_t st, const mhimx_gemm_nt_args& g);
int gemm_tn(hipStream_t st, const mhimx_gemm_tn_args& g);
int layernorm_fwd(hipStream_t st, const float* x, int64_t M, int64_t E, const float* w, const float* b, float* y, float* mean, float* rstd);
int layernorm_bwd(hipStream_t st, const float* dy, const float* x, int64_t M, int64_t E, const float* w, const float* mean,
                  const float* rstd, float* dx, float* dw_part, float* db_part, float* d_w, float* d_b, int accumulate,
                  int max_parts, const float* dy2, const float* x2, const float* mean2, const float* rstd2, int64_t M2,
                  mhimx_reduce_list* defer, const int64_t* xrows = nullptr, const float* resid = nullptr);
int skinny_pair(hipStream_t st, const mhimx_gemm_tn_args& t, const mhimx_gemm_nt_args& g, float a_drop_p = 0.f, uint64_t a_seed = 0,
                const uint64_t* a_tick = nullptr, float* a_colsum = nullptr, int a_accumulate = 0, int use_a_drop = 0);
bool mca_fused_ok(int64_t E, int64_t heads, int64_t dh, int64_t k, const float* wkv_frag, const float* xn, const float* KV);
int mca_fused_fwd(hipStream_t st, const float* xn, int64_t R, const float* wkv_frag, const float* Q, int kq, int heads, float scale,
                  float drop_p, uint64_t seed, const uint64_t* tick, float* KV, float* dots, float* pm, float* pl, float* po);
int colsum(hipStream_t st, const float* X, int64_t M, int64_t E, float* out, int accumulate, void* ws, int64_t ws_bytes);
bool merge2_ok(const mhimx_merge* m, int64_t R);
int64_t merge2_ws_bytes(int64_t R, int64_t k);
int merge2_fwd(hipStream_t st, const mhimx_merge* m, const float* X, int64_t R, float* z, float* q_new, int update_q, void* ws, int64_t ws_bytes);
int merge2_fwd_part(hipStream_t st, const mhimx_merge* m, const float* X, int64_t R, float* part, void* ws, int64_t ws_bytes);
int merge2_fwd_finish(hipStream_t st, const mhimx_merge* m, const float* parts, int W, int64_t R, float* z, float* q_new, int update_q, void* ws,
                      int64_t ws_bytes);
int64_t merge2_part_floats();
int merge2_bwd_park(const mhimx_merge* m, const float* X, int64_t R, const float* dz, float* dX, const mhimx_merge_grad* gr, void* ws, int64_t ws_bytes);
int merge2_bwd(hipStream_t st, const mhimx_merge* m, const float* X, int64_t R, const float* dz, float* dX, const mhimx_merge_grad* gr, void* ws,
               int64_t ws_bytes);

constexpr int MCA_THREADS = 256;
#ifdef MHIMX_MCA_PROF
__device__ unsigned long long mca_prof[16];
#define MCA_STAMP(i) do { __syncthreads(); if (threadIdx.x == 0 && blockIdx.x == 100) mca_prof[i] = wall_clock64(); } while (0)
extern "C" int mhimx_mca_prof_read(unsigned long long* out) { return (int)hipMemcpyFromSymbol(out, HIP_SYMBOL(mca_prof), 16 * 8); }
#else
#define MCA_STAMP(i)
#endif

MHIMX_DEV float block_reduce_sum(float v, float* red ) {
  v = wave_sum(v);
  __syncthreads();
  if ((threadIdx.x & 63) == 0) red[threadIdx.x >> 6] = v;
  __syncthreads();
  return red[0] + red[1] + red[2] + red[3];
}
MHIMX_DEV float block_reduce_max(float v, float* red) {
  v = wave_max(v);
  __syncthreads();
  if ((threadIdx.x & 63) == 0) red[threadIdx.x >> 6] = v;
  __syncthreads();
  return fmaxf(fmaxf(red[0], red[1]), fmaxf(red[2], red[3]));
}

constexpr int MCA_ROWS = 4;
constexpr int MCA_HPW = 2;

template <int KQ>
__global__ __launch_bounds__(MCA_THREADS) void mca_fwd_part_kernel(const float* __restrict__ KV, const float* __restrict__ Q,
                                                                   int64_t R, int heads, int kq, float scale, float drop_p,
                                                                   uint64_t seed0, const uint64_t* __restrict__ tick, float* __restrict__ dots,
                                                                   float* __restrict__ pm, float* __restrict__ pl,
                                                                   float* __restrict__ po) {
  MCA_STAMP(0);
  const uint64_t seed = eff_seed(seed0, tick);
  const int lane = threadIdx.x & 63, wave = threadIdx.x >> 6;
  const int inner = heads * 64;
  const float keep_scale = drop_p > 0.f ? 1.f / (1.f - drop_p) : 1.f;
  float q[MCA_HPW][KQ], m[MCA_HPW][KQ], l[MCA_HPW][KQ], o[MCA_HPW][KQ];
#pragma unroll
  for (int hh = 0; hh < MCA_HPW; ++hh)
#pragma unroll
    for (int i = 0; i < KQ; ++i) {
      const int h = wave + 4 * hh;
      q[hh][i] = (h < heads && i < kq) ? Q[(int64_t)i * inner + h * 64 + lane] * scale : 0.f;
// ... 510 lines not shown
  hipLaunchKernelGGL(mca_reduce_kernel, dim3((unsigned)cdiv(k * I, 64)), dim3(64, 4), 0, st, w.pdq, w.nb, (int)(k * I), w.dQ);
  MHIMX_LAUNCH_CHECK();
  g = {};
  g.A = w.dKV; g.lda = 2 * I; g.B = m->wkv_t; g.ldb = 2 * I; g.C = w.dxn; g.ldc = E; g.M = R; g.N = E; g.K = 2 * I; g.prec = gprec;
  g.ws = w.nt_ws; g.ws_floats = w.nt_ws_floats;
  if (int r = gemm_nt(st, g)) return r;
  t = {};
  t.A = w.dKV; t.lda = 2 * I; t.B = w.xn; t.ldb = E; t.C = gr->d_wkv; t.ldc = E; t.M = R; t.K1 = 2 * I; t.K2 = E;
  t.splits = 1; t.ws = w.scratch; t.ws_floats = w.scratch_bytes / 4; t.accumulate = acc; t.prec = gprec;
  t.defer = gr->defer;
  if (int r = gemm_tn(st, t)) return r;
  t = {};
  t.A = w.dQ; t.lda = I; t.B = w.gq; t.ldb = E; t.C = gr->d_wq; t.ldc = E; t.M = k; t.K1 = I; t.K2 = E; t.splits = 1;
  t.accumulate = acc; t.prec = gprec;
  g = {};
  g.A = w.dQ; g.lda = I; g.B = m->wq_t; g.ldb = I; g.C = w.dgq; g.ldc = E; g.M = k; g.N = E; g.K = I; g.prec = gprec;
  if (int r = skinny_pair(st, t, g)) return r;
  if (R > 16) {
    if (int r = layernorm_bwd(st, w.dxn, X, R, E, m->ln_w, w.mean, w.rstd, dX, w.lnp_w, w.lnp_b, gr->d_ln_w, gr->d_ln_b, acc, 256, w.dgq,
                              m->q_param, w.gmean, w.grstd, k, gr->defer, m->x_rows)) return r;
  } else {
    if (int r = layernorm_bwd(st, w.dxn, X, R, E, m->ln_w, w.mean, w.rstd, dX, w.lnp_w, w.lnp_b, gr->d_ln_w, gr->d_ln_b, acc, 256, nullptr,
                              nullptr, nullptr, nullptr, 0, nullptr, m->x_rows)) return r;
    if (int r = layernorm_bwd(st, w.dgq, m->q_param, k, E, m->ln_w, w.gmean, w.grstd, nullptr, w.lnp_w, w.lnp_b, gr->d_ln_w, gr->d_ln_b, 1, 256,
                              nullptr, nullptr, nullptr, nullptr, 0, nullptr)) return r;
  }
  return 0;
}

}

using namespace mhimx;

extern "C" int mhimx_dropout_apply(void* stream, const float* x, float* out, int64_t M, int64_t E, float p, uint64_t seed,
                                   const uint64_t* tick) {
  MHIMX_CHECK_ARG(x && out && M >= 0 && E > 0 && p >= 0.f && p < 1.f, "dropout_apply: bad args");
  if (M == 0) return 0;
  hipLaunchKernelGGL(drop_bwd_kernel, dim3((unsigned)(cdiv(M * E, 256) < 4096 ? cdiv(M * E, 256) : 4096)), dim3(256), 0, (hipStream_t)stream, x,
                     out, M, (int)E, p, seed, tick);
  MHIMX_LAUNCH_CHECK();
  return 0;
}

extern "C" int64_t mhimx_merge_ws_bytes(int64_t R, int64_t E, int64_t k, int64_t heads, int64_t dim_head) {
  Arena ar(nullptr, 0);
  const int64_t a = merge_ws_layout(ar, R, E, k, heads, dim_head, nullptr);
  const int64_t b = (E == 512 && heads == 8 && dim_head == 64 && heads * k <= 48) ? merge2_ws_bytes(R, k) : 0;
  return a > b ? a : b;
}
extern "C" int mhimx_merge_fwd(void* stream, const mhimx_merge* m, const float* X, int64_t R, float* z, float* q_new,
                               int32_t update_q, void* ws, int64_t ws_bytes) {
  return merge_fwd((hipStream_t)stream, m, X, R, z, q_new, update_q, ws, ws_bytes);
}
extern "C" int64_t mhimx_merge_part_floats(void) { return merge2_part_floats(); }
extern "C" int mhimx_merge_fwd_part(void* stream, const mhimx_merge* m, const float* X, int64_t R, float* part, void* ws, int64_t ws_bytes) {
  if (int r = check_merge(m)) return r;
  MHIMX_CHECK_ARG(X && R > 0 && ws && merge2_ok(m, R), "merge_fwd_part: needs the projection-free form (E = 512, 8 x 64, k <= 6, R <= 32768, not exact f32)");
  return merge2_fwd_part((hipStream_t)stream, m, X, R, part, ws, ws_bytes);
}
extern "C" int mhimx_merge_fwd_finish(void* stream, const mhimx_merge* m, const float* parts, int32_t W, int64_t R, float* z, float* q_new,
                                      int32_t update_q, void* ws, int64_t ws_bytes) {
  if (int r = check_merge(m)) return r;
  MHIMX_CHECK_ARG(R > 0 && ws && merge2_ok(m, R), "merge_fwd_finish: needs the projection-free form");
  return merge2_fwd_finish((hipStream_t)stream, m, parts, W, R, z, q_new, update_q, ws, ws_bytes);
}
extern "C" int mhimx_merge_bwd_park(const mhimx_merge* m, const float* X, int64_t R, const float* dz, float* dX, const mhimx_merge_grad* g, void* ws,
                                    int64_t ws_bytes) {
  if (check_merge(m)) return 0;
  if (!(X && dz && dX && g && R > 0 && g->d_ln_w && g->d_ln_b && g->d_wkv && g->d_wq && g->d_wo && g->d_bo && m->wo_t)) return 0;
  if (!merge2_ok(m, R) || m->own_n != 0) return 0;
  return merge2_bwd_park(m, X, R, dz, dX, g, ws, ws_bytes);
}
extern "C" int mhimx_merge_bwd(void* stream, const mhimx_merge* m, const float* X, int64_t R, const float* dz, float* dX,
                               const mhimx_merge_grad* g, void* ws, int64_t ws_bytes) {
  return merge_bwd((hipStream_t)stream, m, X, R, dz, dX, g, ws, ws_bytes);
}
```

mhim_mil_amd/csrc/mca2.hip:

```cpp
#include <math.h>
#include <string.h>

#include "mca2_rows.hpp"

namespace mhimx {

int64_t merge2_part_floats() { return M2_PART_FLOATS; }
int64_t merge2_rows_tiles(int64_t R) { return cdiv(R, m2_tile_rows(R)); }
int64_t merge2_ws_bytes(int64_t R, int64_t k) {
  Arena ar(nullptr, 0);
  return merge2_ws_layout(ar, R, k, nullptr);
}

bool merge2_ok(const mhimx_merge* m, int64_t R) {
  return m->E == M2_E && m->heads == M2_H && m->dim_head == M2_DH && m->k >= 1 && m->heads * m->k <= M2_JP && R >= 1 && R <= 32768 &&
         m->prec != MHIMX_PREC_F32 && aligned16(m->wq) && aligned16(m->wkv) && aligned16(m->wo) && aligned16(m->ln_w) && aligned16(m->ln_b) &&
         aligned16(m->q_param);
}

__global__ __launch_bounds__(M2_THREADS) void merge2_prep_kernel(Merge2PrepArgs a) {
  __shared__ __attribute__((aligned(16))) float lds[6 * M2_E + 6 * 64];
  merge2_prep_body((int)blockIdx.x, lds, a.q_param, a.ln_w, a.ln_b, a.wq, a.wkv, a.k, a.scale, a.w);
}

template <int RT>
__global__ __launch_bounds__(M2_THREADS) void merge2_rows_fwd_kernel(const float* __restrict__ X, const int64_t* __restrict__ xrows, int64_t R,
                                                                    const float* __restrict__ ln_w, const float* __restrict__ ln_b, int J,
                                                                    float drop_p, uint64_t seed0, const uint64_t* __restrict__ tick, Merge2Ws w, BagBatch bb) {
  extern __shared__ __attribute__((aligned(16))) float m2sm[];
  if (blockIdx.z) {
    MHIMX_BAG(X); MHIMX_BAG(xrows);
    seed0 = bag_mca_seed(seed0, bb);
    bag_move(w, bb);
  }
  merge2_rows_fwd_body<RT>((int)blockIdx.x, m2sm, X, xrows, R, ln_w, ln_b, J, drop_p, seed0, tick, w);
}

template <int MODE>
__global__ __launch_bounds__(M2_THREADS) void merge2_partials_kernel(M2Parts in, int live_only, const float* __restrict__ ln_w,
                                                                    const float* __restrict__ ln_b, float* __restrict__ out,
                                                                    float* __restrict__ stats, float* __restrict__ raw_stats, BagBatch bb) {
  __shared__ float lds[M2_PARTIALS_LDS];
  if (blockIdx.z) {
    in.pm = bag_ptr(in.pm, bb); in.pl = bag_ptr(in.pl, bb); in.psd = bag_ptr(in.psd, bb); in.y = bag_ptr(in.y, bb);
    MHIMX_BAG(out); MHIMX_BAG(stats); MHIMX_BAG(raw_stats);
  }
  merge2_partials_body<MODE>((int)blockIdx.x, lds, in, live_only != 0, ln_w, ln_b, out, stats, raw_stats);
}

__global__ __launch_bounds__(M2_THREADS) void merge2_o_kernel(const float* __restrict__ wkv, int k, Merge2Ws w, BagBatch bb) {
  __shared__ __attribute__((aligned(16))) float ys[6 * M2_E];
  bag_move(w, bb);
  const int tid = threadIdx.x;
  const int h = blockIdx.x >> 2, qd = blockIdx.x & 3;
  M2HeadRows wr;
  m2_head_rows_load<16>(wkv + (int64_t)(M2_I + h * 64 + qd * 16) * M2_E, wr);
  m2_zero_tail(ys, k);
  for (int idx = tid; idx < k * (M2_E / 4); idx += M2_THREADS)
    reinterpret_cast<m2_f4*>(ys)[idx] = reinterpret_cast<const m2_f4*>(w.Y + (int64_t)h * k * M2_E)[idx];
  __syncthreads();
  m2_head_dots_use<16>(wr, ys, k, nullptr, 16, w.O + h * 64 + qd * 16);
}

__global__ __launch_bounds__(M2_THREADS) void merge2_bwd_pre_kernel(const float* __restrict__ dz, const float* __restrict__ wo_t,
                                                                   const float* __restrict__ wkv, int k, float drop_p, uint64_t seed0,
                                                                   const uint64_t* __restrict__ tick, float* __restrict__ d_bo, int accumulate,
                                                                   Merge2Ws w, float rep, BagBatch bb) {
  __shared__ __attribute__((aligned(16))) float lds[M2_BWD_PRE_LDS];
  if (blockIdx.z) {
    MHIMX_BAG(dz); MHIMX_BAG(wo_t); MHIMX_BAG(d_bo);
    seed0 = bag_mca_seed(seed0, bb);
    bag_move(w, bb);
  }
  merge2_bwd_pre_body((int)blockIdx.x, lds, dz, wo_t, wkv, k, drop_p, seed0, tick, d_bo, accumulate, w, rep);
}

template <int RT>
__global__ __launch_bounds__(M2_THREADS) void merge2_rows_bwd_kernel(const float* __restrict__ X, const int64_t* __restrict__ xrows, int64_t R,
                                                                    const float* __restrict__ ln_w, const float* __restrict__ ln_b, int J,
                                                                    float drop_p, uint64_t seed0, const uint64_t* __restrict__ tick,
                                                                    float* __restrict__ dX, Merge2Ws w, BagBatch bb) {
  extern __shared__ __attribute__((aligned(16))) float m2sm[];
  if (blockIdx.z) {
    MHIMX_BAG(X); MHIMX_BAG(xrows); MHIMX_BAG(dX);
    seed0 = bag_mca_seed(seed0, bb);
    bag_move(w, bb);
  }
  merge2_rows_bwd_body<RT>((int)blockIdx.x, m2sm, X, xrows, R, ln_w, ln_b, J, drop_p, seed0, tick, dX, w);
}

__global__ __launch_bounds__(M2_THREADS) void merge2_grads1_kernel(Merge2Side a, BagBatch bb) {
  __shared__ __attribute__((aligned(16))) float lds[M2_GRADS1_LDS];
  bag_move(a, bb);
  merge2_grads1_body((int)blockIdx.x, lds, a);
}

__global__ __launch_bounds__(M2_THREADS) void merge2_grads2_kernel(Merge2Side a, BagBatch bb) {
  __shared__ __attribute__((aligned(16))) float lds[M2_GRADS2_LDS];
  bag_move(a, bb);
  merge2_grads2_body((int)blockIdx.x, lds, a);
}

int mca_out(hipStream_t st, const float* O, const float* wo, const float* bo, int k, int E, int I, float p, uint64_t seed0, const uint64_t* tick,
            float* z, const float* q, float* q_new, float mm);
int reduce_parts2(hipStream_t st, const float* part0, const float* part1, int G, int W, int ld, float* out0, float* out1, int accumulate);

int merge2_side_launch(hipStream_t st, int stage, const Merge2Side& sd) {
  if (stage == 1) hipLaunchKernelGGL(merge2_partials_kernel<0>, bgrid((unsigned)(sd.J * 4)), dim3(M2_THREADS), 0, st, m2_parts_tiles(sd.w, sd.w.upart),
                                     sd.w.own_n > 0 ? 1 : 0, sd.ln_w, sd.ln_b, const_cast<float*>(sd.U), (float*)nullptr, (float*)nullptr, cur_batch());
  else if (stage == 2) hipLaunchKernelGGL(merge2_grads1_kernel, bgrid(M2_GRADS1_BLOCKS), dim3(M2_THREADS), 0, st, sd, cur_batch());
  else hipLaunchKernelGGL(merge2_grads2_kernel, bgrid(M2_GRADS2_BLOCKS), dim3(M2_THREADS), 0, st, sd, cur_batch());
  MHIMX_LAUNCH_CHECK();
  return 0;
}
int merge2_side_finish(hipStream_t st, mhimx_side_work* side, int upto_stage) {
  Merge2Side sd;
  while (side->pending != 0 && side->pending <= upto_stage) {
    memcpy(&sd, side->blob, sizeof(sd));
    if (int r = merge2_side_launch(st, side->pending, sd)) return r;
    side->pending = side->pending == 3 ? 0 : side->pending + 1;
  }
  return 0;
}

int merge2_fwd_rows_args(const mhimx_merge* m, const float* X, int64_t R, void* ws, int64_t ws_bytes, M2RowsFwd* out) {
  if (!m || !X || !merge2_ok(m, R) || !m->prepared || m->own_n != 0) return 1;
  Arena ar(ws, ws_bytes);
  Merge2Ws w;
  merge2_ws_layout(ar, R, m->k, &w);
  MHIMX_CHECK_ARG(ar.ok(), "merge rows rider: workspace too small (%lld < %lld)", (long long)ws_bytes, (long long)ar.off);
  if (w.rt != 16) return 1;
  w.own_lo = 0; w.own_n = 0;
  *out = M2RowsFwd{X, m->x_rows, R, m->ln_w, m->ln_b, M2_H * (int)m->k, m->drop_p, m->drop_seed, m->drop_tick, w};
  return 0;
}

static int merge2_fwd_rows(hipStream_t st, const mhimx_merge* m, const float* X, int64_t R, void* ws, int64_t ws_bytes, Merge2Ws* wout) {
  Arena ar(ws, ws_bytes);
  Merge2Ws w;
  merge2_ws_layout(ar, R, m->k, &w);
  MHIMX_CHECK_ARG(ar.ok(), "merge_fwd: workspace too small (%lld < %lld)", (long long)ws_bytes, (long long)ar.off);
  MHIMX_CHECK_ARG(m->own_n >= 0 && (m->own_n == 0 || m->x_rows), "merge_fwd: a shard's row range needs the bag-level row list (x_rows)");
  w.own_lo = m->own_n > 0 ? m->own_lo : 0;
  w.own_n = m->own_n;
  const int k = (int)m->k, J = M2_H * k;
  const float scale = 1.0f / sqrtf((float)M2_DH);
  if (m->rows_done) {
    *wout = w;
    return 0;
  }
  if (!m->prepared) {
    hipLaunchKernelGGL(merge2_prep_kernel, dim3(64), dim3(M2_THREADS), 0, st, Merge2PrepArgs{m->q_param, m->ln_w, m->ln_b, m->wq, m->wkv, k, scale, w});
    MHIMX_LAUNCH_CHECK();
  }
  MHIMX_ONCE_PER_DEVICE(MHIMX_HIP(hipFuncSetAttribute((const void*)merge2_rows_fwd_kernel<32>, hipFuncAttributeMaxDynamicSharedMemorySize, (int)m2_fwd_smem(32)));
                        MHIMX_HIP(hipFuncSetAttribute((const void*)merge2_rows_fwd_kernel<16>, hipFuncAttributeMaxDynamicSharedMemorySize, (int)m2_fwd_smem(16))));
  if (w.rt == 16)
    hipLaunchKernelGGL(merge2_rows_fwd_kernel<16>, bgrid((unsigned)w.T), dim3(M2_THREADS), m2_fwd_smem(16), st, X, m->x_rows, R, m->ln_w, m->ln_b, J, m->drop_p,
                       m->drop_seed, m->drop_tick, w, cur_batch());
  else
    hipLaunchKernelGGL(merge2_rows_fwd_kernel<32>, bgrid((unsigned)w.T), dim3(M2_THREADS), m2_fwd_smem(32), st, X, m->x_rows, R, m->ln_w, m->ln_b, J, m->drop_p,
                       m->drop_seed, m->drop_tick, w, cur_batch());
  MHIMX_LAUNCH_CHECK();
  *wout = w;
  return 0;
}
static int merge2_fwd_tail(hipStream_t st, const mhimx_merge* m, float* z, float* q_new, int update_q, const Merge2Ws& w) {
  const int k = (int)m->k;
  hipLaunchKernelGGL(merge2_o_kernel, bgrid(M2_H * 4), dim3(M2_THREADS), 0, st, m->wkv, k, w, cur_batch());
  MHIMX_LAUNCH_CHECK();
  return mca_out(st, w.O, m->wo, m->bo, k, M2_E, M2_I, m->drop_p, m->drop_seed + 0x9E3779B97F4A7C15ull, m->drop_tick, z, m->q_param,
                 update_q ? q_new : (float*)nullptr, m->mm);
}

int merge2_fwd(hipStream_t st, const mhimx_merge* m, const float* X, int64_t R, float* z, float* q_new, int update_q, void* ws, int64_t ws_bytes) {
  MHIMX_CHECK_ARG(!update_q || q_new, "merge_fwd: update_q needs q_new");
  MHIMX_CHECK_ARG(m->own_n == 0, "merge_fwd: a shard of an instance-sharded bag runs mhimx_merge_fwd_part + mhimx_merge_fwd_finish");
  Merge2Ws w;
  if (int r = merge2_fwd_rows(st, m, X, R, ws, ws_bytes, &w)) return r;
  const int J = M2_H * (int)m->k;
  hipLaunchKernelGGL(merge2_partials_kernel<1>, bgrid((unsigned)(J * 4)), dim3(M2_THREADS), 0, st, m2_parts_tiles(w, w.ypart), 0, m->ln_w, m->ln_b, w.Y,
                     w.stats, (float*)nullptr, cur_batch());
  MHIMX_LAUNCH_CHECK();
  return merge2_fwd_tail(st, m, z, q_new, update_q, w);
}

int merge2_fwd_part(hipStream_t st, const mhimx_merge* m, const float* X, int64_t R, float* part, void* ws, int64_t ws_bytes) {
  MHIMX_CHECK_ARG(part && aligned16(part), "merge_fwd_part: null / unaligned output block");
  Merge2Ws w;
  if (int r = merge2_fwd_rows(st, m, X, R, ws, ws_bytes, &w)) return r;
  const int J = M2_H * (int)m->k;
  hipLaunchKernelGGL(merge2_partials_kernel<2>, dim3((unsigned)(J * 4)), dim3(M2_THREADS), 0, st, m2_parts_tiles(w, w.ypart), 0, m->ln_w, m->ln_b,
                     part + 3 * M2_JP, (float*)nullptr, part, BagBatch{});
  MHIMX_LAUNCH_CHECK();
  return 0;
}
int merge2_fwd_finish(hipStream_t st, const mhimx_merge* m, const float* parts, int W, int64_t R, float* z, float* q_new, int update_q, void* ws,
                      int64_t ws_bytes) {
  MHIMX_CHECK_ARG(parts && W >= 1 && W <= 256 && z, "merge_fwd_finish: 1..256 shard blocks");
  MHIMX_CHECK_ARG(!update_q || q_new, "merge_fwd_finish: update_q needs q_new");
  Arena ar(ws, ws_bytes);
  Merge2Ws w;
  merge2_ws_layout(ar, R, m->k, &w);
  MHIMX_CHECK_ARG(ar.ok(), "merge_fwd_finish: workspace too small");
  const int J = M2_H * (int)m->k;
  hipLaunchKernelGGL(merge2_partials_kernel<1>, dim3((unsigned)(J * 4)), dim3(M2_THREADS), 0, st, m2_parts_shards(parts, W), 0, m->ln_w, m->ln_b, w.Y,
                     w.stats, (float*)nullptr, BagBatch{});
  MHIMX_LAUNCH_CHECK();
  return merge2_fwd_tail(st, m, z, q_new, update_q, w);
}

int gemm_tn_rider(hipStream_t st, const mhimx_gemm_tn_args& g, const Merge2Side* rider, int stage);

static int merge2_side_of(const mhimx_merge* m, const float* X, int64_t R, const float* dz, float* dX, const mhimx_merge_grad* gr, void* ws,
                          int64_t ws_bytes, Merge2Side* out) {
  Arena ar(ws, ws_bytes);
  Merge2Ws w;
  merge2_ws_layout(ar, R, m->k, &w);
  MHIMX_CHECK_ARG(ar.ok(), "merge_bwd: workspace too small");
  MHIMX_CHECK_ARG(m->own_n >= 0 && (m->own_n == 0 || m->x_rows), "merge_bwd: a shard's row range needs the bag-level row list (x_rows)");
  w.own_lo = m->own_n > 0 ? m->own_lo : 0;
  w.own_n = m->own_n;
  MHIMX_CHECK_ARG(m->wo_t && aligned16(m->wo_t), "merge_bwd: transposed to_out weight missing");
  const int k = (int)m->k, J = M2_H * k;
  Merge2Side sd = {};
  sd.w = w; sd.dz = dz; sd.U = w.aq; sd.ln_w = m->ln_w; sd.ln_b = m->ln_b; sd.wkv = m->wkv; sd.wq = m->wq; sd.q_param = m->q_param; sd.wo_t = m->wo_t;
  sd.d_wkv = gr->d_wkv; sd.d_wo = gr->d_wo; sd.d_wq = gr->d_wq; sd.d_ln_w = gr->d_ln_w; sd.d_ln_b = gr->d_ln_b; sd.d_bo = gr->d_bo; sd.tick = m->drop_tick;
  sd.oseed = m->drop_seed + 0x9E3779B97F4A7C15ull; sd.scale = 1.0f / sqrtf((float)M2_DH); sd.drop_p = m->drop_p; sd.k = k; sd.accumulate = gr->accumulate;
  sd.J = J;
  sd.rep = m->own_n > 0 ? m->rep : 1.f;
  sd.X = X; sd.xrows = m->x_rows; sd.R = R; sd.dX = dX; sd.seed0 = m->drop_seed;
  *out = sd;
  return 0;
}

int merge2_bwd_park(const mhimx_merge* m, const float* X, int64_t R, const float* dz, float* dX, const mhimx_merge_grad* gr, void* ws, int64_t ws_bytes) {
  if (!gr->defer || gr->defer->pre.pending != 0) return 0;
  Merge2Side sd;
  if (int r = merge2_side_of(m, X, R, dz, dX, gr, ws, ws_bytes, &sd)) return r;
  static_assert(sizeof(Merge2Side) <= sizeof(gr->defer->pre.blob), "Merge2Side must fit mhimx_reduce_list.pre");
  memcpy(gr->defer->pre.blob, &sd, sizeof(sd));
  gr->defer->pre.pending = 1;
  return 0;
}

int merge2_bwd(hipStream_t st, const mhimx_merge* m, const float* X, int64_t R, const float* dz, float* dX, const mhimx_merge_grad* gr, void* ws,
               int64_t ws_bytes) {
  Merge2Side sd;
  if (int r = merge2_side_of(m, X, R, dz, dX, gr, ws, ws_bytes, &sd)) return r;
  const Merge2Ws& w = sd.w;
  const int k = sd.k, J = sd.J;
  const int acc = gr->accumulate;
  const uint64_t oseed = sd.oseed;
  bool pre_done = false, rows_done = false;
  if (gr->defer && gr->defer->pre.pending) {
    pre_done = gr->defer->pre.pending == 2;
    gr->defer->pre.pending = 0;
  }
  if (gr->defer && gr->defer->parked.pending) {
    mhimx_gemm_tn_args pg;
    memcpy(&pg, gr->defer->parked.blob, sizeof(pg));
    gr->defer->parked.pending = 0;
    if (pre_done) {
      const int rc = gemm_tn_rider(st, pg, &sd, 4);
      if (rc < 0) return rc;
      rows_done = rc == 1;
    } else {
      const int rc = gemm_tn_rider(st, pg, pre_done ? nullptr : &sd, 0);
      if (rc < 0) return rc;
      pre_done = pre_done || rc == 1;
    }
  }
  if (!pre_done) {
    hipLaunchKernelGGL(merge2_bwd_pre_kernel, bgrid(M2_BWD_PRE_BLOCKS), dim3(M2_THREADS), 0, st, dz, m->wo_t, m->wkv, k, m->drop_p, oseed, m->drop_tick, gr->d_bo, acc, w, sd.rep, cur_batch());
    MHIMX_LAUNCH_CHECK();
  }
  if (!rows_done) {
    MHIMX_ONCE_PER_DEVICE(MHIMX_HIP(hipFuncSetAttribute((const void*)merge2_rows_bwd_kernel<32>, hipFuncAttributeMaxDynamicSharedMemorySize, (int)m2_bwd_smem(32)));
                          MHIMX_HIP(hipFuncSetAttribute((const void*)merge2_rows_bwd_kernel<16>, hipFuncAttributeMaxDynamicSharedMemorySize, (int)m2_bwd_smem(16))));
    if (w.rt == 16)
      hipLaunchKernelGGL(merge2_rows_bwd_kernel<16>, bgrid((unsigned)w.T), dim3(M2_THREADS), m2_bwd_smem(16), st, X, m->x_rows, R, m->ln_w, m->ln_b, J, m->drop_p,
                         m->drop_seed, m->drop_tick, dX, w, cur_batch());
    else
      hipLaunchKernelGGL(merge2_rows_bwd_kernel<32>, bgrid((unsigned)w.T), dim3(M2_THREADS), m2_bwd_smem(32), st, X, m->x_rows, R, m->ln_w, m->ln_b, J, m->drop_p,
                         m->drop_seed, m->drop_tick, dX, w, cur_batch());
    MHIMX_LAUNCH_CHECK();
  }
  if (gr->defer && gr->defer->side.pending == 0) {
    memcpy(gr->defer->side.blob, &sd, sizeof(sd));
    gr->defer->side.pending = 1;
  } else {
    for (int stage = 1; stage <= 3; ++stage)
      if (int r = merge2_side_launch(st, stage, sd)) return r;
  }
  return 0;
}

}

namespace mhimx {
int merge2_prep_args(const mhimx_merge* m, int64_t R, void* ws, int64_t ws_bytes, Merge2PrepArgs* out) {
  MHIMX_CHECK_ARG(m && merge2_ok(m, R), "prep_batch: the Merge preparation job needs the projection-free form (E = 512, 8 x 64, k <= 6, R <= 32768)");
  Arena ar(ws, ws_bytes);
  Merge2Ws w;
  merge2_ws_layout(ar, R, m->k, &w);
  MHIMX_CHECK_ARG(ar.ok(), "prep_batch: Merge workspace too small (%lld < %lld)", (long long)ws_bytes, (long long)ar.off);
  *out = Merge2PrepArgs{m->q_param, m->ln_w, m->ln_b, m->wq, m->wkv, (int)m->k, 1.0f / sqrtf((float)M2_DH), w};
  return 0;
}
}
```

mhim_mil_amd/csrc/mca2_prep.hpp:

```cpp
#pragma once

#include "mma_tile.hpp"

namespace mhimx {

constexpr int M2_E = 512, M2_H = 8, M2_DH = 64, M2_I = 512, M2_JP = 48, M2_JK = 64, M2_ROWS = 32, M2_THREADS = 256;
constexpr int M2_XLD = M2_E + 4;
constexpr int M2_PLD = 36;
constexpr int M2_CLD = 2 * M2_JK + 4;

typedef float m2_f4 __attribute__((ext_vector_type(4)));

struct Merge2Ws {
  float *gq, *gmean, *grstd, *Q, *aq, *aqf, *gtf_aq, *mean, *rstd, *S, *pm, *pl, *psd, *ypart, *stats, *Y, *O;
  float *dO, *dyf, *gtf_dy, *dpart, *upart, *lnpart, *dQ;
  unsigned* gate;
  int64_t own_lo, own_n;
  int T;
  int rt;
};

MHIMX_DEV void bag_move(Merge2Ws& w, const BagBatch& bb) {
  if (blockIdx.z == 0) return;
#define M2_MV(f) w.f = bag_ptr(w.f, bb)
  M2_MV(gq); M2_MV(gmean); M2_MV(grstd); M2_MV(Q); M2_MV(aq); M2_MV(aqf); M2_MV(gtf_aq); M2_MV(mean); M2_MV(rstd); M2_MV(S); M2_MV(pm); M2_MV(pl);
  M2_MV(psd); M2_MV(ypart); M2_MV(stats); M2_MV(Y); M2_MV(O); M2_MV(dO); M2_MV(dyf); M2_MV(gtf_dy); M2_MV(dpart); M2_MV(upart); M2_MV(lnpart);
  M2_MV(dQ); M2_MV(gate);
#undef M2_MV
}

inline int m2_tile_rows(int64_t R) {
  return R <= 4096 ? 16 : 32;
}

inline int64_t merge2_ws_layout(Arena& ar, int64_t R, int64_t k, Merge2Ws* out) {
  Merge2Ws w;
  w.rt = m2_tile_rows(R);
  const int64_t T = cdiv(R, w.rt);
  w.T = (int)T;
  w.gq = ar.take<float>(k * M2_E);
  w.gmean = ar.take<float>(k);
  w.grstd = ar.take<float>(k);
  w.Q = ar.take<float>(k * M2_I);
  w.aq = ar.take<float>(M2_JP * M2_E);
  w.aqf = ar.take<float>(3 * 16 * 64 * 8);
  w.gtf_aq = ar.take<float>(32 * 2 * 64 * 8);
  w.mean = ar.take<float>(R);
  w.rstd = ar.take<float>(R);
  w.S = ar.take<float>(R * M2_JP);
  w.pm = ar.take<float>(T * M2_JP);
  w.pl = ar.take<float>(T * M2_JP);
  w.psd = ar.take<float>(T * M2_JP);
  w.ypart = ar.take<float>(T * M2_JP * M2_E);
  w.stats = ar.take<float>(M2_JP * 2);
  w.Y = ar.take<float>(M2_JP * M2_E);
  w.O = ar.take<float>(k * M2_I);
  w.dO = ar.take<float>(k * M2_I);
  w.dyf = ar.take<float>(3 * 16 * 64 * 8);
  w.gtf_dy = ar.take<float>(32 * 2 * 64 * 8);
  w.dpart = ar.take<float>(M2_JP * 8);
  w.upart = ar.take<float>(T * M2_JP * M2_E);
  w.lnpart = ar.take<float>(T * 2 * M2_E);
  w.dQ = ar.take<float>(k * M2_I);
  w.gate = reinterpret_cast<unsigned*>(ar.take<float>(64));
  w.own_lo = 0; w.own_n = 0;
  if (out) *out = w;
  return ar.off;
}

MHIMX_DEV void m2_split8(const float (&v)[8], bf8& hi, bf8& lo) {
#pragma unroll
  for (int i = 0; i < 8; ++i) {
    const __bf16 h = (__bf16)v[i];
    hi[i] = h;
    lo[i] = (__bf16)(v[i] - (float)h);
  }
}
MHIMX_DEV f32x4 m2_mfma(const bf8& a, const bf8& b, const f32x4& c) { return __builtin_amdgcn_mfma_f32_16x16x32_bf16(a, b, c, 0, 0, 0); }
MHIMX_DEV f32x4 m2_mfma3(const bf8& ah, const bf8& al, const bf8& bh, const bf8& bl, f32x4 c) {
  c = m2_mfma(al, bh, c);
  c = m2_mfma(ah, bl, c);
  return m2_mfma(ah, bh, c);
}
MHIMX_DEV void m2_load_frag(const float* img, int entry, int lane, bf8& hi, bf8& lo) {
  const m2_f4* p = reinterpret_cast<const m2_f4*>(img + ((int64_t)entry * 64 + lane) * 8);
  hi = __builtin_bit_cast(bf8, p[0]);
  lo = __builtin_bit_cast(bf8, p[1]);
}
MHIMX_DEV void m2_store_images(float* f, float* gtf, int j, int e, float v) {
  const __bf16 h = (__bf16)v, l = (__bf16)(v - (float)h);
  if (j < M2_JP) {
    __bf16* p = reinterpret_cast<__bf16*>(f) + (((int64_t)((j >> 4) * 16 + (e >> 5)) * 64 + ((e & 31) >> 3) * 16 + (j & 15)) * 16) + (e & 7);
// ... 59 lines not shown
MHIMX_DEV void m2_head_dots(const float* __restrict__ rows, const float* vec, int k, float* out, int out_ld, float* gout) {
  M2HeadRows r;
  m2_head_rows_load<NR>(rows, r);
  m2_head_dots_use<NR>(r, vec, k, out, out_ld, gout);
}
MHIMX_DEV void m2_zero_tail(float* v, int k) {
  for (int idx = k * M2_E + threadIdx.x; idx < 6 * M2_E; idx += M2_THREADS) v[idx] = 0.f;
}

MHIMX_DEV void merge2_prep_body(int block, float* lds, const float* __restrict__ q_param, const float* __restrict__ ln_w, const float* __restrict__ ln_b,
                                const float* __restrict__ wq, const float* __restrict__ wkv, int k, float scale, const Merge2Ws& w) {
  float* gqs = lds;
  float* qh = gqs + 6 * M2_E;
  const int tid = threadIdx.x, lane = tid & 63, wave = tid >> 6;
  const int h = block >> 3, eb = block & 7;
  const int J = M2_H * k;
  const int c = tid & 63, e = eb * 64 + c;
  float wv[64];
#pragma unroll
  for (int d = 0; d < 64; ++d) wv[d] = wkv[(int64_t)(h * 64 + d) * M2_E + e];
  m2_zero_tail(gqs, k);
  for (int idx = k * 64 + tid; idx < 6 * 64; idx += M2_THREADS) qh[idx] = 0.f;
  for (int i = wave; i < k; i += 4) {
    const float* row = q_param + (int64_t)i * M2_E;
    const m2_f4 a = *reinterpret_cast<const m2_f4*>(row + 4 * lane), b = *reinterpret_cast<const m2_f4*>(row + 256 + 4 * lane);
    float mu, rs;
    m2_ln_stats(a, b, mu, rs);
    const m2_f4 wa = *reinterpret_cast<const m2_f4*>(ln_w + 4 * lane), wb = *reinterpret_cast<const m2_f4*>(ln_w + 256 + 4 * lane);
    const m2_f4 ba = *reinterpret_cast<const m2_f4*>(ln_b + 4 * lane), bb = *reinterpret_cast<const m2_f4*>(ln_b + 256 + 4 * lane);
    const m2_f4 ya = (a - mu) * rs * wa + ba, yb = (b - mu) * rs * wb + bb;
    *reinterpret_cast<m2_f4*>(gqs + i * M2_E + 4 * lane) = ya;
    *reinterpret_cast<m2_f4*>(gqs + i * M2_E + 256 + 4 * lane) = yb;
    if (block == 0) {
      *reinterpret_cast<m2_f4*>(w.gq + i * M2_E + 4 * lane) = ya;
      *reinterpret_cast<m2_f4*>(w.gq + i * M2_E + 256 + 4 * lane) = yb;
      if (lane == 0) { w.gmean[i] = mu; w.grstd[i] = rs; }
    }
  }
  __syncthreads();
  m2_head_dots<64>(wq + (int64_t)h * 64 * M2_E, gqs, k, qh, 64, eb == 0 ? w.Q + h * 64 : nullptr);
  __syncthreads();
  for (int i = tid >> 6; i < k; i += 4) {
    float acc = 0.f;
#pragma unroll
    for (int d = 0; d < 64; ++d) acc += qh[i * 64 + d] * wv[d];
    acc *= scale;
    const int j = h * k + i;
    m2_store_images(w.aqf, w.gtf_aq, j, e, acc);
  }
  for (int j = J + h; j < M2_JK; j += M2_H)
    if ((tid >> 6) == ((j - J) >> 3) % 4) m2_store_images(w.aqf, w.gtf_aq, j, e, 0.f);
}


struct Merge2PrepArgs { const float *q_param, *ln_w, *ln_b, *wq, *wkv; int k; float scale; Merge2Ws w; };

}
```

mhim_mil_amd/csrc/prep_jobs.hpp:

```cpp
#pragma once
#include "mma_tile.hpp"
#include "mca2_prep.hpp"

namespace mhimx {

typedef float pj_f4 __attribute__((ext_vector_type(4)));
typedef __bf16 pj_b8 __attribute__((ext_vector_type(8)));
MHIMX_DEV void pj_split(const float (&x)[8], pj_b8& hi, pj_b8& lo) {
#pragma unroll
  for (int i = 0; i < 8; ++i) {
    const __bf16 h = (__bf16)x[i];
    hi[i] = h;
    lo[i] = (__bf16)(x[i] - (float)h);
  }
}
MHIMX_DEV void pj_split2(const pj_f4& a, const pj_f4& b, pj_b8& hi, pj_b8& lo) {
  const float x[8] = {a[0], a[1], a[2], a[3], b[0], b[1], b[2], b[3]};
  pj_split(x, hi, lo);
}

constexpr int PREP_MERGE_MAX = 8;
struct PrepJobs { mhimx_prep_job j[MHIMX_PREP_MAX]; int first[MHIMX_PREP_MAX + 1]; int n; Merge2PrepArgs m2; int64_t m2_shift[PREP_MERGE_MAX]; };
constexpr int PREP_LDS_FLOATS = 6 * M2_E + 6 * 64;
static_assert(PREP_LDS_FLOATS >= 32 * 33, "the transpose tile fits the job LDS");
// ... 71 lines not shown
      const float* src = jb.in + 8 * g8 * C + m;
      float x[8];
#pragma unroll
      for (int u = 0; u < 8; ++u) x[u] = src[u * C];
      pj_b8 hi, lo;
      pj_split(x, hi, lo);
      pj_f4* o = reinterpret_cast<pj_f4*>(jb.out + (m * R8 + g8) * 8);
      o[0] = __builtin_bit_cast(pj_f4, hi);
      o[1] = __builtin_bit_cast(pj_f4, lo);
    }
  } else if (jb.kind == 8) {
    const int64_t KS = C / 32, NB = (R + 15) / 16, n = NB * KS * 64;
    for (int64_t i = (int64_t)bid * 256 + threadIdx.x; i < n; i += (int64_t)nblk * 256) {
      const int64_t lane = i & 63, ks = (i >> 6) % KS, nb = (i >> 6) / KS;
      const int64_t row = 16 * nb + (lane & 15);
      pj_f4 a = {0.f, 0.f, 0.f, 0.f}, b = a;
      if (row < R) {
        const float* src = jb.in + row * C + 32 * ks + 8 * (lane >> 4);
        a = *reinterpret_cast<const pj_f4*>(src);
        b = *reinterpret_cast<const pj_f4*>(src + 4);
      }
      pj_b8 hi, lo;
      pj_split2(a, b, hi, lo);
      pj_f4* o = reinterpret_cast<pj_f4*>(jb.out + i * 8);
      o[0] = __builtin_bit_cast(pj_f4, hi);
      o[1] = __builtin_bit_cast(pj_f4, lo);
    }
  } else if (jb.kind == 9) {
    const int64_t nJ = C / 256, ntiles = ((R + 31) / 32) * nJ;
    const int koct = threadIdx.x >> 6, q = threadIdx.x & 63;
    for (int64_t t = bid; t < ntiles; t += nblk) {
      const int64_t ks = t / nJ, cb = t % nJ, r0 = ks * 32 + koct * 8;
      const float* src = jb.in + r0 * C + cb * 256 + 4 * q;
      pj_f4 v[8];
#pragma unroll
      for (int u = 0; u < 8; ++u) v[u] = r0 + u < R ? *reinterpret_cast<const pj_f4*>(src + u * C) : pj_f4{0.f, 0.f, 0.f, 0.f};
      char* tile = reinterpret_cast<char*>(jb.out) + t * 32768 + ((koct * 2) * 256 + q) * 16;
#pragma unroll
      for (int j = 0; j < 4; ++j) {
        const float x[8] = {v[0][j], v[1][j], v[2][j], v[3][j], v[4][j], v[5][j], v[6][j], v[7][j]};
        pj_b8 hi, lo;
        pj_split(x, hi, lo);
        *reinterpret_cast<pj_f4*>(tile + j * 1024) = __builtin_bit_cast(pj_f4, hi);
        *reinterpret_cast<pj_f4*>(tile + j * 1024 + 4096) = __builtin_bit_cast(pj_f4, lo);
      }
    }
  } else if (jb.kind == 10) {
    int64_t* o = reinterpret_cast<int64_t*>(jb.out);
    for (int64_t i = (int64_t)bid * 256 + threadIdx.x; i < C; i += (int64_t)nblk * 256) o[i] = R + i;
  } else if (jb.kind == 6) {
    Merge2Ws w = pj.m2.w;
    const int64_t sh = pj.m2_shift[jb.R];
    w.gq += sh; w.gmean += sh; w.grstd += sh; w.Q += sh; w.aq += sh; w.aqf += sh; w.gtf_aq += sh; w.gate += sh;
    merge2_prep_body(bid, lds, pj.m2.q_param, pj.m2.ln_w, pj.m2.ln_b, pj.m2.wq, pj.m2.wkv, pj.m2.k, pj.m2.scale, w);
  }
}

int prep_jobs_fill(const mhimx_prep_job* jobs, int n, PrepJobs* out);
int prep_batch(hipStream_t st, const mhimx_prep_job* jobs, int n);

}
```

mhim_mil_amd/csrc/ragged_window.hip:

```cpp
#include <math.h>
#include <string.h>

#include "infer_tab.hpp"
#include "step_mid.hpp"
#include "surv_dev.hpp"

namespace mhimx {

namespace {

constexpr int RW_ROWS = RG_ROWS, RW_T = 256;
constexpr int FIN_SCORE_BLOCKS = 8;
constexpr int RW_MAX = MHIMX_RAGGED_WINDOW_MAX;

typedef _Float16 rw_h4 __attribute__((ext_vector_type(4)));

struct RwCnt { int32_t len_keep[RW_MAX]; int32_t slot[RW_MAX]; };

__global__ __launch_bounds__(RW_T) void rw_pad_kernel(InferTab tab, RwCnt cn, float* __restrict__ Ht, float* __restrict__ Hs,
                                                      _Float16* __restrict__ dact, uint8_t* __restrict__ keep) {
  const int bag = blockIdx.x;
  int64_t N = tab.N[0], orow0 = tab.row0[0];
  int slot = cn.slot[0];
  RG_PICK(N, tab.N, bag) RG_PICK(orow0, tab.row0, bag) RG_PICK(slot, cn.slot, bag)
// ... 249 lines not shown
  out->H_teacher = w.H_t; out->H_student = w.H_s; out->dact = w.dact; out->dpre = w.dH; out->z_teacher = w.z_t; out->z_student = w.z_s;
  return 0;
}

extern "C" int mhimx_ragged_window_run(void* stream, const mhimx_step_cfg* cfg, int32_t n_bags, const mhimx_ragged_window_bag* bags,
                                       int64_t host_step, void* ws, int64_t ws_bytes, int32_t update) {
  return mhimx_ragged_window_run_x(stream, cfg, n_bags, bags, host_step, ws, ws_bytes, update, MHIMX_X_F32);
}

extern "C" int mhimx_ragged_window_run_x(void* stream, const mhimx_step_cfg* cfg, int32_t n_bags, const mhimx_ragged_window_bag* bags,
                                         int64_t host_step, void* ws, int64_t ws_bytes, int32_t update, int32_t x_dtype) {
  return mhimx::ragged_window_run(stream, cfg, n_bags, bags, host_step, ws, ws_bytes, update, x_dtype, nullptr);
}

extern "C" int mhimx_ragged_window_run_surv(void* stream, const mhimx_step_cfg* cfg, int32_t n_bags, const mhimx_ragged_window_bag* bags,
                                            int64_t host_step, void* ws, int64_t ws_bytes, int32_t update, int32_t x_dtype,
                                            const mhimx_surv_spec* surv) {
  MHIMX_CHECK_ARG(surv, "ragged_window: null survival description (mhimx_ragged_window_run_x is the classification call)");
  return mhimx::ragged_window_run(stream, cfg, n_bags, bags, host_step, ws, ws_bytes, update, x_dtype, surv);
}

int mhimx::ragged_window_run(void* stream, const mhimx_step_cfg* cfg, int32_t n_bags, const mhimx_ragged_window_bag* bags, int64_t host_step,
                             void* ws, int64_t ws_bytes, int32_t update, int32_t x_dtype, const mhimx_surv_spec* surv) {
  if (int r = check_rw(cfg, n_bags, bags, x_dtype)) return r;
  if (surv)
    if (int r = surv_spec_check("ragged_window", n_bags, surv)) return r;
  for (int b = 0; b < n_bags; ++b) {
    MHIMX_CHECK_ARG(bags[b].X && aligned16(bags[b].X), "ragged_window: bag %d: null or unaligned rows", b);
    MHIMX_CHECK_ARG(bags[b].label_dev, "ragged_window: bag %d: null label", b);
  }
  MHIMX_CHECK_ARG(!update || (cfg->p && cfg->g && cfg->m && cfg->v && cfg->n_train > 0 && cfg->n_all >= cfg->n_train),
                  "ragged_window: update needs the flat optimiser buffers");
  RwLay w;
  InferTab tab = {};
  RwCnt cn = {};
  rw_layout(cfg, n_bags, bags, &w, &tab, &cn, nullptr);
  tab.pad = x_dtype;
  if (int r = rg_check_ws("ragged_window", ws, ws_bytes, w.total)) return r;
  const mhimx_step_cfg& c = *cfg;
  const mhimx_step_params &S = c.student, &T = c.teacher;
  const int64_t D = c.D, E = c.E, C = c.C, k = c.k;
  hipStream_t st = (hipStream_t)stream;
  char* base = static_cast<char*>(ws);
  auto F = [&](int64_t off) { return reinterpret_cast<float*>(base + off); };
  const MidImages im = {F(w.w1p_t), F(w.wa_frag_t), F(w.w1p_s), F(w.wa_frag_s), F(w.wa_t), F(w.wa_t_frag), F(w.wo_t), F(w.q_old)};
  float *H_t = F(w.H_t), *H_s = F(w.H_s), *dHall = F(w.dH), *s_t = F(w.s_t), *score_all = F(w.score), *cproj = F(w.cproj);
  _Float16* dact = reinterpret_cast<_Float16*>(base + w.dact);
  int64_t* rows_space = reinterpret_cast<int64_t*>(base + w.rows_all);
  uint8_t* keep = reinterpret_cast<uint8_t*>(base + w.keep);
  void* merge_ws = base + w.merge_ws;
  const uint64_t* tick = c.tick;

  const mhimx_merge mw_prep = mid_merge_params(c);
  {
    mhimx_prep_job jobs[10];
    int n = mid_prep_head(c, im, jobs);
    n += mid_prep_student(c, im, jobs + n);
    if (int r = mhimx_prep_batch(stream, jobs, n)) return r;
  }
  {
    PureWinDrop dr = {};
    dr.tick = tick; dr.dact = dact;
    for (int b = 0; b < n_bags; ++b) dr.seed[b] = bags[b].seeds.drop_teacher;
    dr.drop_p = c.drop_p_teacher;
    if (int r = pure_window_project(st, tab, dr, (int)D, im.w1p_t, T.b1, c.act, H_t)) return r;
    for (int b = 0; b < n_bags; ++b) dr.seed[b] = bags[b].seeds.drop_student;
    dr.drop_p = c.drop_p_student;
    if (int r = pure_window_project(st, tab, dr, (int)D, im.w1p_s, S.b1, c.act, H_s)) return r;
  }
  hipLaunchKernelGGL(rw_pad_kernel, dim3((unsigned)n_bags, 4), dim3(RW_T), 0, st, tab, cn, H_t, H_s, dact, keep);
  MHIMX_LAUNCH_CHECK();
  if (c.attn2score) {
    if (int r = infer_score_cproj(st, tab, H_t, im.wa_frag_t, T.wc, c.da_act, s_t, F(w.pm), F(w.pl), F(w.pz), T.wp, (int)C, cproj)) return r;
  } else if (int r = infer_score(st, tab, H_t, im.wa_frag_t, T.wc, c.da_act, s_t, F(w.pm), F(w.pl), F(w.pz)))
    return r;
  hipLaunchKernelGGL(rw_finalize_kernel, dim3((unsigned)n_bags, 1 + FIN_SCORE_BLOCKS), dim3(RG_FIN_T), 0, st, tab, F(w.pm), F(w.pl), F(w.pz), s_t, cproj, T.bp,
                     (int)C, (int)c.attn2score, F(w.z_t), F(w.stats_t), score_all);
  MHIMX_LAUNCH_CHECK();
  {
    mhimx_select_bag sb[RW_MAX];
    for (int b = 0; b < n_bags; ++b) {
      const mhimx_step_counts& cnt = bags[b].cnt;
      sb[b] = mhimx_select_bag{tab.row0[b], bags[b].N, cnt.k_top, cnt.n_sel, cnt.R, tab.row0[b], bags[b].seeds.select};
    }
    SelLargeWs lw;
    lw.perm = reinterpret_cast<int64_t*>(base + w.sel_perm); lw.ids = reinterpret_cast<int64_t*>(base + w.sel_ids);
    lw.rows = reinterpret_cast<int64_t*>(base + w.sel_rows); lw.lk = reinterpret_cast<int64_t*>(base + w.sel_lk);
    lw.sel_ws = base + w.sel_ws; lw.sel_ws_bytes = w.sel_ws_bytes;
    if (int r = select_bags_check("ragged_window", n_bags, sb)) return r;
    if (int r = select_rows_many_launch(st, score_all, n_bags, sb, tick, rows_space, lw, 1)) return r;
  }

  const float inv_n = 1.f / (float)n_bags;
  for (int b = 0; b < n_bags; ++b) {
    const mhimx_ragged_window_bag& g = bags[b];
    const int64_t N = g.N, R = g.cnt.R, row0 = tab.row0[b];
    int64_t* rows_all = rows_space + row0;
    const int acc = b > 0 ? 1 : 0;
    {
      mhimx_prep_job jobs[2];
      jobs[0] = mhimx_prep_job{10, nullptr, reinterpret_cast<float*>(rows_all + g.cnt.len_keep), N, k};
      jobs[1] = mhimx_prep_job{6, reinterpret_cast<const float*>(&mw_prep), static_cast<float*>(merge_ws), R, w.merge_ws_bytes};
      if (int r = mhimx_prep_batch(stream, jobs, 2)) return r;
    }
    const MidBag mb = {H_s + row0 * E, dHall + row0 * E, rows_all, N, R, g.cnt.Lk, g.seeds.mca, F(w.q_scr), F(w.s_s), F(w.stats_s), F(w.z_s) + (int64_t)b * E,
                       F(w.g_z), base + w.pool_ws_s, w.pool_ws_s_bytes, merge_ws, w.merge_ws_bytes};
    MidFwd fwd;
    if (int r = mid_student_fwd(stream, c, im, mw_prep, mb, nullptr, &fwd)) return r;
    const MidSurv sv = {surv ? surv->censor_dev[b] : nullptr, surv ? surv->alpha : 0.f, surv ? surv->eps : 0.f, surv && surv->risk ? surv->risk + b : nullptr};
    if (int r = mid_head(stream, c, mb, F(w.z_t) + (int64_t)b * E, g.label_dev, inv_n, F(w.logits) + 16 * b, F(w.losses) + 4 * b, c.grad, acc,
                         surv ? &sv : nullptr))
      return r;
    mhimx_reduce_list lst;
    memset(&lst, 0, sizeof(lst));
    if (int r = mid_bwd_rows(stream, im, fwd, mb, c.grad, acc, nullptr, nullptr, &lst)) return r;
    if (int r = mhimx_reduce_flush(stream, &lst)) return r;
  }

  hipLaunchKernelGGL(rw_keep_kernel, dim3((unsigned)n_bags, 8), dim3(RW_T), 0, st, tab, cn, rows_space, keep);
  MHIMX_LAUNCH_CHECK();
  hipLaunchKernelGGL(rw_dpre_kernel, dim3((unsigned)w.steps), dim3(RW_T), 0, st, keep, dHall, dact, F(w.db1_part));
  MHIMX_LAUNCH_CHECK();
  if (int r = pw_wgrad_bagx(st, tab, dHall, (int)D, w.steps, w.s1, w.s1_per, F(w.slab_1))) return r;
  {
    const float* parts[2] = {F(w.slab_1), F(w.db1_part)};
    const int32_t G[2] = {w.s1, w.steps};
    const int64_t W[2] = {E * D, E};
    float* out[2] = {c.grad.w1, c.grad.b1};
    if (int r = pw_reduce(st, 2, parts, G, W, out)) return r;
  }
  {
    int64_t tok[RW_MAX];
    for (int b = 0; b < n_bags; ++b) tok[b] = tab.row0[b] + bags[b].N;
    if (int r = rw_q_chain(st, S.q, H_s, n_bags, tok, (double)c.merge_mm, (int)(k * E))) return r;
  }
  if (!update) return 0;
  const mhimx_optim_args o = optim_args_of(c, host_step, true);
  return mhimx_optim_step(stream, &o);
}
```

mhim_mil_amd/csrc/step.hip:

```cpp
#include <math.h>
#include <string.h>

#include "infer_tab.hpp"
#include "step_mid.hpp"

namespace mhimx {

int64_t merge2_rows_tiles(int64_t R);

namespace {

struct DagEvents {
  hipEvent_t e[64][6];
  bool have[64] = {};
  int get(hipEvent_t** out) {
    int dev = 0;
    MHIMX_HIP(hipGetDevice(&dev));
    MHIMX_CHECK_ARG(dev >= 0 && dev < 64, "step: device index %d", dev);
    if (!have[dev]) {
      for (int i = 0; i < 6; ++i) MHIMX_HIP(hipEventCreateWithFlags(&e[dev][i], hipEventDisableTiming));
      have[dev] = true;
    }
    *out = e[dev];
    return 0;
// ... 450 lines not shown
    MHIMX_CHECK_ARG(gp[i] >= c->g && gp[i] < c->g + c->n_train, "window: every gradient view lies inside the flat gradient buffer g[0, n_train)");
  MHIMX_CHECK_ARG(g.w1 == c->g && (c->E * c->D) % 4 == 0, "window: feature.0.weight's gradient is the FIRST block of the flat gradient buffer");
  for (int i = 1; i < 12; ++i) MHIMX_CHECK_ARG(gp[i] >= c->g + c->E * c->D, "window: gradient views overlap feature.0.weight's");
  return 0;
}

}
}

extern "C" int mhimx_window_layout_of(const mhimx_step_cfg* cfg, int32_t n_bags, int64_t N, const mhimx_step_counts* cnt, mhimx_window_layout* out) {
  MHIMX_CHECK_ARG(out, "window_layout: null output");
  if (int r = check_window(cfg, n_bags, N, cnt)) return r;
  StepBufs b;
  layout(cfg, N, cnt, &b, n_bags);
  out->total = b.total; out->bag0 = b.bag0; out->bag_stride = b.bag_stride; out->grad_slab = b.gslab;
  out->bag = mhimx_step_layout{b.total, b.logits, b.losses, cfg->attn2score ? b.pscore : b.attn, b.rows_all, b.H_t, b.Hbuf, b.dact, b.z_t, b.z_s, b.g_z, b.dH};
  return 0;
}

extern "C" int mhimx_window_run(void* stream, const mhimx_step_cfg* cfg, int32_t n_bags, const float* const* X, int64_t ldx, int64_t N,
                                const int64_t* const* labels_dev, const mhimx_step_counts* cnt, const mhimx_step_seeds* seeds, int64_t host_step, void* ws,
                                int64_t ws_bytes, int32_t update) {
  if (int r = check_window(cfg, n_bags, N, cnt)) return r;
  MHIMX_CHECK_ARG(X && labels_dev && seeds && ws && ldx >= cfg->D && ldx % 4 == 0 && N * ldx * 4 < ((int64_t)1 << 32),
                  "window: null bags / labels / seeds / workspace, or a row pitch the weight-gradient product does not take");
  for (int32_t i = 0; i < n_bags; ++i) MHIMX_CHECK_ARG(X[i] && aligned16(X[i]) && labels_dev[i], "window: bag %d / its label null or not 16-byte aligned", i);
  MHIMX_CHECK_ARG(!update || (cfg->p && cfg->m && cfg->v), "window: update needs the flat optimiser buffers");
  StepBufs b;
  layout(cfg, N, cnt, &b, n_bags);
  MHIMX_CHECK_ARG(ws_bytes >= b.total && (reinterpret_cast<uintptr_t>(ws) & 255) == 0, "window: workspace too small (%lld < %lld) or not 256-byte aligned",
                  (long long)ws_bytes, (long long)b.total);
  const mhimx_step_cfg& c = *cfg;
  const mhimx_step_params &S = c.student, &T = c.teacher;
  const int64_t D = c.D, E = c.E, A = c.A, C = c.C, k = c.k, I = 512;
  const int64_t R = cnt->R, Lk = cnt->Lk, len_keep = cnt->len_keep;
  const hipStream_t st = (hipStream_t)stream;
  Carve cv(ws);
  const int64_t BS = b.bag_stride;
  auto bag = [&](int64_t off, int i) { return cv.at<char>(off) + (int64_t)i * BS; };
  const MidImages im = {cv.at<float>(b.w1p_t), cv.at<float>(b.wa_frag_t), cv.at<float>(b.w1p_s), cv.at<float>(b.wa_frag_s),
                        cv.at<float>(b.wa_t),  cv.at<float>(b.wa_t_frag), cv.at<float>(b.wo_t),  cv.at<float>(b.q_old)};
  float* H_t = cv.at<float>(b.H_t);
  float* Hbuf = cv.at<float>(b.Hbuf);
  void* dact = cv.at<char>(b.dact);
  int64_t* rows_all = cv.at<int64_t>(b.rows_all);
  float* dH = cv.at<float>(b.dH);
  float* slab0 = cv.at<float>(b.gslab);
  const uint64_t* tick = c.tick;
  auto gs = [&](float* view) { return slab0 + (view - c.g); };

  const int64_t g_lo = E * D;

  const mhimx_merge mw_prep = mid_merge_params(c);
  {
    mhimx_prep_job jobs[MHIMX_PREP_MAX];
    int n = mid_prep_head(c, im, jobs);
    n += mid_prep_student(c, im, jobs + n);
    for (int i = 0; i < n_bags; ++i) {
      jobs[n++] = mhimx_prep_job{10, nullptr, reinterpret_cast<float*>(reinterpret_cast<int64_t*>(bag(b.rows_all, i)) + len_keep), N, k};
      jobs[n++] = mhimx_prep_job{6, reinterpret_cast<const float*>(&mw_prep), reinterpret_cast<float*>(bag(b.merge_ws, i)), R, b.merge_ws_bytes};
    }
    static_assert(10 + 2 * MHIMX_WINDOW_MAX <= MHIMX_PREP_MAX, "the window's preparation is one launch");
    if (int r = mhimx_prep_batch(stream, jobs, n)) return r;
  }

  {
    mhimx_bag_project_args pa[MHIMX_WINDOW_MAX];
    for (int i = 0; i < n_bags; ++i) {
      mhimx_bag_project_args a = {};
      a.X = X[i]; a.ldx = ldx; a.N = N; a.D = D; a.E = E; a.act = c.act; a.n_heads = 2; a.drop_tick = tick;
      a.head[0].wp = im.w1p_t; a.head[0].bias = T.b1; a.head[0].H = reinterpret_cast<float*>(bag(b.H_t, i)); a.head[0].ldh = E; a.head[0].drop_p = c.drop_p_teacher;
      a.head[0].drop_seed = seeds[i].drop_teacher;
      a.head[1].wp = im.w1p_s; a.head[1].bias = S.b1; a.head[1].H = reinterpret_cast<float*>(bag(b.Hbuf, i)); a.head[1].ldh = E; a.head[1].dact = bag(b.dact, i);
      a.head[1].drop_p = c.drop_p_student; a.head[1].drop_seed = seeds[i].drop_student;
      pa[n_bags - 1 - i] = a;
    }
    if (int r = mhimx_bag_project_multi(stream, pa, n_bags)) return r;
  }

  BagBatch bb = {};
  bb.n = n_bags;
  bb.lo[0] = reinterpret_cast<uint64_t>(cv.at<char>(b.bag0)); bb.span[0] = (uint64_t)BS; bb.stride[0] = BS;
  bb.tab_key = reinterpret_cast<uint64_t>(labels_dev[0]);
  for (int i = 0; i < n_bags; ++i) {
    bb.dsel[i] = seeds[i].select - seeds[0].select;
    bb.dmca[i] = seeds[i].mca - seeds[0].mca;
    bb.tab[i] = reinterpret_cast<uint64_t>(labels_dev[i]);
  }
  struct BatchScope {
    explicit BatchScope(const BagBatch* p) { set_batch(p); }
    ~BatchScope() { set_batch(nullptr); }
  };
  {
    BatchScope scope(&bb);
    const mhimx_scorer sc_t = mid_scorer(c, T, im.wa_frag_t);
    const float* score = nullptr;
    {
      mhimx_pool_io io = {};
      io.T1 = H_t; io.M1 = N; io.s = cv.at<float>(b.s_t); io.stats = cv.at<float>(b.stats_t); io.z = cv.at<float>(b.z_t);
      io.ws = cv.at<char>(b.pool_ws_t); io.ws_bytes = b.pool_ws_t_bytes;
      if (c.attn2score) { io.wp = T.wp; io.C = C; io.cproj = cv.at<float>(b.cproj_t); io.bp = T.bp; io.pscore = cv.at<float>(b.pscore); }
      io.no_backward = 1;
      if (int r = mhimx_abmil_pool_fwd(stream, &sc_t, &io)) return r;
      if (c.attn2score) score = io.pscore;
      else {
        if (int r = mhimx_softmax_from_stats(stream, io.s, io.stats, cv.at<float>(b.attn), N)) return r;
        score = cv.at<float>(b.attn);
      }
    }
    if (int r = mhimx_select_rows_img(stream, score, N, cnt->k_top, cnt->n_sel, 1, seeds[0].select, tick, R, rows_all, cv.at<int64_t>(b.rows_img), b.P0,
                                      cv.at<char>(b.sel_ws), b.sel_ws_bytes, 1))
      return r;
    const MidBag g = {Hbuf, dH, rows_all, N, R, Lk, seeds[0].mca, cv.at<float>(b.q_scr), cv.at<float>(b.s_s), cv.at<float>(b.stats_s), cv.at<float>(b.z_s),
// ... 236 lines not shown
```

mhim_mil_amd/ops.py:

```python
from __future__ import annotations

import ctypes as C
from typing import Optional

import torch

from . import _lib as L


KERNEL_EVENT_HOOK = None


import threading

_PIN = threading.local()


def _pinned():
    st = getattr(_PIN, "stream", None)
    if st is not None and getattr(_PIN, "device", -1) == torch.cuda.current_device():
        return st
    return None


# ... 445 lines not shown

def random_perm(n, seed, tick=None, src=None, out=None, device=None):
    _chk(src, torch.int64, "src"); _chk(out, torch.int64, "out")
    dev = device if device is not None else (src.device if src is not None else (out.device if out is not None else torch.device("cuda")))
    if out is None:
        out = torch.empty(int(n), dtype=torch.int64, device=dev)
    L.check(L.lib().mhimx_random_perm(_stream(), int(n), int(seed) & 0xFFFFFFFFFFFFFFFF, _p(tick), _p(src), _p(out)), "mhimx_random_perm")
    return out


def compose_ids(a, b):
    _chk(a, torch.int64, "a"); _chk(b, torch.int64, "b")
    out = torch.empty_like(b)
    L.check(L.lib().mhimx_compose_ids(_stream(), _p(a), _p(b), _p(out), b.numel()), "mhimx_compose_ids")
    return out


class MergeW:
    def __init__(self, q_param, ln_w, ln_b, wkv, wq, wo, bo, mm, heads=8, dim_head=64, drop_p=0.0, drop_seed=0,
                 prec="bf16x3", transposes=None, drop_tick=None, wkv_frag=None, x_rows=None, prepared=False, own=None, rep=1.0):
        self.t = [q_param, ln_w, ln_b, wkv, wq, wo, bo, wkv_frag]
        _chk(x_rows, torch.int64, "x_rows")
        self.x_rows = x_rows
        for t in self.t:
            _chk(t, name="merge weight")
        self.k, self.E = q_param.shape[-2], q_param.shape[-1]
        self.heads, self.dim_head = heads, dim_head
        self.tr = transposes or (None, None, None)
        self.c = L.Merge(E=self.E, k=self.k, heads=heads, dim_head=dim_head, q_param=_p(q_param), ln_w=_p(ln_w),
                         ln_b=_p(ln_b), wkv=_p(wkv), wq=_p(wq), wo=_p(wo), bo=_p(bo), wkv_t=_p(self.tr[0]),
                         wq_t=_p(self.tr[1]), wo_t=_p(self.tr[2]), mm=float(mm), drop_p=float(drop_p),
                         drop_seed=int(drop_seed) & 0xFFFFFFFFFFFFFFFF, prec=prec_code(prec), drop_tick=_p(drop_tick),
                         wkv_frag=_p(wkv_frag), x_rows=_p(x_rows), prepared=int(bool(prepared)),
                         own_lo=0 if own is None else int(own[0]), own_n=0 if own is None else int(own[1]), rep=float(rep))
        self.own = own

    def ws_for(self, R, device):
        n = L.lib().mhimx_merge_ws_bytes(R, self.E, self.k, self.heads, self.dim_head)
        return torch.empty(n, device=device, dtype=torch.uint8)


def merge_fwd(mw: MergeW, X, z_out=None, update_q=True, ws=None, q_out=None, rows_done=False):
    _chk(X, name="X")
    R = X.shape[0] if mw.x_rows is None else mw.x_rows.shape[0]
    dev = X.device
    z = z_out if z_out is not None else torch.empty((mw.k, mw.E), device=dev)
    q_new = (q_out if q_out is not None else torch.empty((mw.k, mw.E), device=dev)) if update_q else None
    ws = ws if ws is not None else mw.ws_for(R, dev)
    mw.c.rows_done = int(bool(rows_done))
    L.check(L.lib().mhimx_merge_fwd(_stream(), C.byref(mw.c), _p(X), R, _p(z), _p(q_new), int(bool(update_q)), _p(ws),
                                    ws.numel()), "mhimx_merge_fwd")
    mw.c.rows_done = 0
    return z, q_new, ws


def merge_fwd_part(mw: MergeW, X, ws=None, part=None):
    _chk(X, name="X")
    R = mw.x_rows.shape[0]
    dev = X.device
    part = part if part is not None else torch.empty(L.lib().mhimx_merge_part_floats(), device=dev)
    ws = ws if ws is not None else mw.ws_for(R, dev)
    L.check(L.lib().mhimx_merge_fwd_part(_stream(), C.byref(mw.c), _p(X), R, _p(part), _p(ws), ws.numel()), "mhimx_merge_fwd_part")
    return part, ws


def merge_fwd_finish(mw: MergeW, parts, ws, z_out=None, update_q=True, q_out=None):
    _chk(parts, name="parts")
    R = mw.x_rows.shape[0]
    dev = parts.device
    z = z_out if z_out is not None else torch.empty((mw.k, mw.E), device=dev)
    q_new = (q_out if q_out is not None else torch.empty((mw.k, mw.E), device=dev)) if update_q else None
    L.check(L.lib().mhimx_merge_fwd_finish(_stream(), C.byref(mw.c), _p(parts), parts.shape[0], R, _p(z), _p(q_new), int(bool(update_q)),
                                           _p(ws), ws.numel()), "mhimx_merge_fwd_finish")
    return z, q_new


def merge_bwd_park(mw: MergeW, X, dz, ws, grads, accumulate=False, defer=None):
    if defer is None or mw.x_rows is None:
        return
    R = mw.x_rows.shape[0]
    g = L.MergeGrad(d_ln_w=_p(grads["d_ln_w"]), d_ln_b=_p(grads["d_ln_b"]), d_wkv=_p(grads["d_wkv"]), d_wq=_p(grads["d_wq"]),
                    d_wo=_p(grads["d_wo"]), d_bo=_p(grads["d_bo"]), accumulate=int(bool(accumulate)), splits=8, defer=_dp(defer))
    L.check(L.lib().mhimx_merge_bwd_park(C.byref(mw.c), _p(X), R, _p(dz), _p(grads["dX"]), C.byref(g), _p(ws), ws.numel()), "mhimx_merge_bwd_park")


def merge_bwd(mw: MergeW, X, dz, ws, splits=8, grads=None, accumulate=False, defer=None):
    dev = X.device
    R, E = X.shape
    if mw.x_rows is not None:
        R = mw.x_rows.shape[0]
        if not grads or "dX" not in grads:
            raise L.MhimxError("merge_bwd with gathered rows scatters into a caller-provided dX buffer")
    I = mw.heads * mw.dim_head
    out = grads or {}
    out.setdefault("dX", torch.empty((R, E), device=dev))
    out.setdefault("d_ln_w", torch.empty(E, device=dev))
    out.setdefault("d_ln_b", torch.empty(E, device=dev))
    out.setdefault("d_wkv", torch.empty((2 * I, E), device=dev))
    out.setdefault("d_wq", torch.empty((I, E), device=dev))
    out.setdefault("d_wo", torch.empty((E, I), device=dev))
    out.setdefault("d_bo", torch.empty(E, device=dev))
    g = L.MergeGrad(d_ln_w=_p(out["d_ln_w"]), d_ln_b=_p(out["d_ln_b"]), d_wkv=_p(out["d_wkv"]), d_wq=_p(out["d_wq"]),
                    d_wo=_p(out["d_wo"]), d_bo=_p(out["d_bo"]), accumulate=int(bool(accumulate)), splits=int(splits),
                    defer=_dp(defer))
    if defer is not None:
        defer.keep.append(ws)
# ... 744 lines not shown
```

Measured before the change: 33.63 million patch-instances/s.

## Premultiply to_out and value weights so merge forward tail runs in fewer launches

Adds a per-head premultiplied matrix Mw = Wo_h · Wv_h (8×512×512), computed once per step by extra blocks in the Merge prep kernel. A new merge2_out_kernel applies Mw directly to Y to produce z and q_new, and runs the O computation in the same launch. This is meant to cut a separate output-projection launch in the merge forward tail. The price is the premultiply work and 8 MB of Mw traffic per bag, with only the first bag's prep job computing Mw and later bags sharing it. It is unclear whether the default merge2_fwd path uses two_launch; only the new API sets it.

```diff
diff --git a/include/mhimx.h b/include/mhimx.h
--- a/include/mhimx.h
+++ b/include/mhimx.h
@@ -282,6 +282,10 @@
 int64_t mhimx_merge_ws_bytes(int64_t R, int64_t E, int64_t k, int64_t heads, int64_t dim_head);
 int mhimx_merge_fwd(void* stream, const mhimx_merge* m, const float* X, int64_t R, float* z, float* q_new,
                     int32_t update_q, void* ws, int64_t ws_bytes);
+int mhimx_merge_fwd_two_launch(void* stream, const mhimx_merge* m, const float* X, int64_t R, float* z, float* q_new,
+                               int32_t update_q, void* ws, int64_t ws_bytes);
+typedef struct { int64_t premul, Y, O; } mhimx_merge_ws_view;
+int mhimx_merge_ws_view_of(int64_t R, int64_t k, mhimx_merge_ws_view* out);
 typedef struct {
   float* d_ln_w; float* d_ln_b; float* d_wkv; float* d_wq; float* d_wo; float* d_bo;
   int32_t accumulate; int32_t splits;
diff --git a/mhim_mil_amd/_lib.py b/mhim_mil_amd/_lib.py
--- a/mhim_mil_amd/_lib.py
+++ b/mhim_mil_amd/_lib.py
@@ -130,6 +130,10 @@
                 ("mm", C.c_float), ("drop_p", C.c_float), ("drop_seed", C.c_uint64), ("prec", C.c_int32), ("drop_tick", C.c_void_p),
                 ("wkv_frag", c_f32p), ("x_rows", c_i64p), ("prepared", C.c_int32), ("own_lo", C.c_int64), ("own_n", C.c_int64),
                 ("rep", C.c_float), ("rows_done", C.c_int32)]
+
+
+class MergeWsView(C.Structure):
+    _fields_ = [("premul", C.c_int64), ("Y", C.c_int64), ("O", C.c_int64)]
 
 
 class MergeGrad(C.Structure):
@@ -364,6 +368,8 @@
     "mhimx_select_rows_many": (C.c_int, [_P, _P, _I32, _P, _P, _P, _P, _I64, _I32]),
     "mhimx_merge_ws_bytes": (_I64, [_I64, _I64, _I64, _I64, _I64]),
     "mhimx_merge_fwd": (C.c_int, [_P, C.POINTER(Merge), _P, _I64, _P, _P, _I32, _P, _I64]),
+    "mhimx_merge_fwd_two_launch": (C.c_int, [_P, C.POINTER(Merge), _P, _I64, _P, _P, _I32, _P, _I64]),
+    "mhimx_merge_ws_view_of": (C.c_int, [_I64, _I64, C.POINTER(MergeWsView)]),
     "mhimx_merge_part_floats": (_I64, []),
     "mhimx_merge_fwd_part": (C.c_int, [_P, C.POINTER(Merge), _P, _I64, _P, _P, _I64]),
     "mhimx_merge_fwd_finish": (C.c_int, [_P, C.POINTER(Merge), _P, _I32, _I64, _P, _P, _I32, _P, _I64]),
diff --git a/mhim_mil_amd/csrc/common.hpp b/mhim_mil_amd/csrc/common.hpp
--- a/mhim_mil_amd/csrc/common.hpp
+++ b/mhim_mil_amd/csrc/common.hpp
@@ -114,6 +114,12 @@
 };
 const BagBatch& cur_batch();
 void set_batch(const BagBatch* b);
+float* cur_premul();
+void set_premul(float* m);
+struct PremulScope {
+  explicit PremulScope(float* m) { set_premul(m); }
+  ~PremulScope() { set_premul(nullptr); }
+};
 inline dim3 bgrid(unsigned x, unsigned y = 1) { return dim3(x, y, cur_batch().n > 0 ? (unsigned)cur_batch().n : 1u); }
 
 #define MHIMX_DEV __device__ __forceinline__
diff --git a/mhim_mil_amd/csrc/dsmil_mhim.hip b/mhim_mil_amd/csrc/dsmil_mhim.hip
--- a/mhim_mil_amd/csrc/dsmil_mhim.hip
+++ b/mhim_mil_amd/csrc/dsmil_mhim.hip
@@ -7,6 +7,7 @@
 
 bool merge2_ok(const mhimx_merge* m, int64_t R);
 int64_t merge2_ws_bytes(int64_t R, int64_t k);
+int64_t merge2_premul_floats();
 
 namespace {
 
@@ -255,7 +256,7 @@
 }
 
 struct DmLay {
-  int64_t w1p_t, w1p_s, vp_t, q0f_t, q2f_t, vp, vtp, q0f, q2f, q2tf, q0tf, wo_t;
+  int64_t w1p_t, w1p_s, vp_t, q0f_t, q2f_t, vp, vtp, q0f, q2f, q2tf, q0tf, wo_t, premul;
   int64_t logits, losses, logits_bag, logits_ins, B, crit, B_t, lb_t, lg_t, li_t, crit_t, qmax_t, qmax, stats, gli, dB, delta, dqmax, dwfcc_part,
       dbfcc_part, dwi_part, dbi_part;
   int64_t H_t, H_s, dact, V_t, Q_t, cls_t, score, rows_all, pos, db1_part, pmax_t, parg_t, pm_t, pl_t, pB_t, slab_1;
@@ -373,6 +374,7 @@
   w->q2tf = ar.off; ar.take<float>(DM_Q * DM_Q);
   w->q0tf = ar.off; ar.take<float>(DM_Q * E);
   w->wo_t = ar.off; ar.take<float>(512 * E);
+  w->premul = ar.off; ar.take<float>(merge2_premul_floats());
   w->logits = ar.off; ar.take<float>(n * C);
   w->losses = ar.off; ar.take<float>(n * 3);
   w->logits_bag = ar.off; ar.take<float>(n * C);
@@ -435,7 +437,7 @@
   w->Xm = ar.off; ar.take<float>(mrows * E);
   w->dXm = ar.off; ar.take<float>(mrows * E);
   for (int b = 0; b < n_bags; ++b) {
-    w->merge_ws_bytes[b] = merge2_ws_bytes(bags[b].cnt.R, k);
+    w->merge_ws_bytes[b] = merge2_ws_bytes(bags[b].cnt.R, k) - merge2_premul_floats() * (int64_t)sizeof(float);
     w->merge_ws[b] = ar.off; ar.take<char>(w->merge_ws_bytes[b]);
   }
   w->sel_ws_bytes = sel_b; w->sel_ws = ar.off; ar.take<char>(sel_b);
@@ -505,6 +507,9 @@
   float* q_dst = cfg->q_out ? cfg->q_out : cfg->q;
 
   mhimx_merge mw_prep = dm_merge_params(*cfg);
+  mhimx_merge mw_prep_later = mw_prep;
+  mw_prep_later.prepared = 1;
+  const PremulScope premul_scope(F(w.premul));
   {
     mhimx_prep_job jobs[24];
     int n = 0;
@@ -524,7 +529,8 @@
     jobs[n++] = mhimx_prep_job{0, cfg->merge.wo, F(w.wo_t), c.E, 512};
     if (cfg->q_out) jobs[n++] = mhimx_prep_job{2, cfg->q, cfg->q_out, 1, k * c.E};
     for (int b = 0; b < n_bags && b < 8; ++b)
-      jobs[n++] = mhimx_prep_job{6, reinterpret_cast<const float*>(&mw_prep), reinterpret_cast<float*>(base + w.merge_ws[b]), bags[b].cnt.R, w.merge_ws_bytes[b]};
+      jobs[n++] = mhimx_prep_job{6, reinterpret_cast<const float*>(b == 0 ? &mw_prep : &mw_prep_later), reinterpret_cast<float*>(base + w.merge_ws[b]),
+                                 bags[b].cnt.R, w.merge_ws_bytes[b]};
     if (int r = mhimx_prep_batch(stream, jobs, n)) return r;
   }
   {
@@ -569,7 +575,7 @@
       mhimx_prep_job jobs[8];
       int n = 0;
       for (int q = b; q < n_bags && q < b + 8; ++q)
-        jobs[n++] = mhimx_prep_job{6, reinterpret_cast<const float*>(&mw_prep), reinterpret_cast<float*>(base + w.merge_ws[q]), bags[q].cnt.R, w.merge_ws_bytes[q]};
+        jobs[n++] = mhimx_prep_job{6, reinterpret_cast<const float*>(&mw_prep_later), reinterpret_cast<float*>(base + w.merge_ws[q]), bags[q].cnt.R, w.merge_ws_bytes[q]};
       if (int r = mhimx_prep_batch(stream, jobs, n)) return r;
     }
     mhimx_merge mw = mw_prep;
diff --git a/mhim_mil_amd/csrc/errors.hip b/mhim_mil_amd/csrc/errors.hip
--- a/mhim_mil_amd/csrc/errors.hip
+++ b/mhim_mil_amd/csrc/errors.hip
@@ -16,6 +16,9 @@
 }
 const std::string& last_error() { return g_err; }
 
+static thread_local float* g_premul = nullptr;
+float* cur_premul() { return g_premul; }
+void set_premul(float* m) { g_premul = m; }
 static thread_local BagBatch g_batch = {};
 const BagBatch& cur_batch() { return g_batch; }
 void set_batch(const BagBatch* b) {
diff --git a/mhim_mil_amd/csrc/gemm_dma.hip b/mhim_mil_amd/csrc/gemm_dma.hip
--- a/mhim_mil_amd/csrc/gemm_dma.hip
+++ b/mhim_mil_amd/csrc/gemm_dma.hip
@@ -497,11 +497,14 @@
       Merge2PrepArgs m2;
       if (int r = merge2_prep_args(reinterpret_cast<const mhimx_merge*>(jobs[i].in), jobs[i].R, jobs[i].out, jobs[i].C, &m2)) return r;
       if (n_merge == 0) pj.m2 = m2;
-      MHIMX_CHECK_ARG(m2.q_param == pj.m2.q_param && m2.wq == pj.m2.wq && m2.wkv == pj.m2.wkv && m2.ln_w == pj.m2.ln_w && m2.k == pj.m2.k,
+      MHIMX_CHECK_ARG(m2.q_param == pj.m2.q_param && m2.wq == pj.m2.wq && m2.wkv == pj.m2.wkv && m2.wo == pj.m2.wo && m2.ln_w == pj.m2.ln_w && m2.k == pj.m2.k,
                       "prep_batch: the Merge preparation jobs of one launch share their parameters");
-      MHIMX_CHECK_ARG((m2.w.gq - pj.m2.w.gq) == (m2.w.gtf_aq - pj.m2.w.gtf_aq), "prep_batch: Merge workspace layouts differ");
+      const bool premul = !reinterpret_cast<const mhimx_merge*>(jobs[i].in)->prepared;
+      MHIMX_CHECK_ARG((m2.w.gq - pj.m2.w.gq) == (m2.w.gtf_aq - pj.m2.w.gtf_aq) && (!premul || (m2.w.gq - pj.m2.w.gq) == (m2.w.Mw - pj.m2.w.Mw)),
+                      "prep_batch: Merge workspace layouts differ");
       pj.m2_shift[n_merge] = m2.w.gq - pj.m2.w.gq;
       pj.j[i].R = n_merge++;
+      pj.j[i].C = premul ? 1 : 0;
     }
     MHIMX_CHECK_ARG(jobs[i].kind != 5 || (jobs[i].C % 32 == 0 && jobs[i].R % 16 == 0 && aligned16(jobs[i].out)),
                     "prep_batch: the transposed fragment image needs C % 32 == 0, R % 16 == 0 and a 16-byte aligned output");
@@ -520,7 +523,7 @@
     const int64_t items = (jobs[i].kind == 3 || jobs[i].kind == 10) ? 1 : (jobs[i].kind == 0 ? cdiv(jobs[i].R, 32) * cdiv(jobs[i].C, 32) :
                           (jobs[i].kind == 8 ? cdiv(jobs[i].R, 16) * 16 * jobs[i].C / 8 : jobs[i].R * jobs[i].C / 8));
     int64_t want = jobs[i].kind == 0 ? items : cdiv(items, 256);
-    if (jobs[i].kind == 6) want = 64;
+    if (jobs[i].kind == 6) want = M2_PREP_BLOCKS + (pj.j[i].C ? M2_PREMUL_ITEMS : 0);
     if (jobs[i].kind == 9) want = cdiv(jobs[i].R, 32) * (jobs[i].C / 256);
     if (want < 1) want = 1;
     if (want > 4096) want = 4096;
diff --git a/mhim_mil_amd/csrc/mca.hip b/mhim_mil_amd/csrc/mca.hip
--- a/mhim_mil_amd/csrc/mca.hip
+++ b/mhim_mil_amd/csrc/mca.hip
@@ -19,7 +19,9 @@
 int colsum(hipStream_t st, const float* X, int64_t M, int64_t E, float* out, int accumulate, void* ws, int64_t ws_bytes);
 bool merge2_ok(const mhimx_merge* m, int64_t R);
 int64_t merge2_ws_bytes(int64_t R, int64_t k);
-int merge2_fwd(hipStream_t st, const mhimx_merge* m, const float* X, int64_t R, float* z, float* q_new, int update_q, void* ws, int64_t ws_bytes);
+int merge2_fwd(hipStream_t st, const mhimx_merge* m, const float* X, int64_t R, float* z, float* q_new, int update_q, void* ws, int64_t ws_bytes,
+               int two_launch = 0);
+void merge2_ws_view(int64_t R, int64_t k, int64_t* out);
 int merge2_fwd_part(hipStream_t st, const mhimx_merge* m, const float* X, int64_t R, float* part, void* ws, int64_t ws_bytes);
 int merge2_fwd_finish(hipStream_t st, const mhimx_merge* m, const float* parts, int W, int64_t R, float* z, float* q_new, int update_q, void* ws,
                       int64_t ws_bytes);
@@ -636,6 +638,19 @@
                                int32_t update_q, void* ws, int64_t ws_bytes) {
   return merge_fwd((hipStream_t)stream, m, X, R, z, q_new, update_q, ws, ws_bytes);
 }
+extern "C" int mhimx_merge_fwd_two_launch(void* stream, const mhimx_merge* m, const float* X, int64_t R, float* z, float* q_new, int32_t update_q,
+                                          void* ws, int64_t ws_bytes) {
+  if (int r = check_merge(m)) return r;
+  MHIMX_CHECK_ARG(X && z && R > 0 && ws && merge2_ok(m, R), "merge_fwd_two_launch: needs the projection-free form (E = 512, 8 x 64, k <= 6, R <= 32768, not exact f32)");
+  return merge2_fwd((hipStream_t)stream, m, X, R, z, q_new, update_q, ws, ws_bytes, 1);
+}
+extern "C" int mhimx_merge_ws_view_of(int64_t R, int64_t k, mhimx_merge_ws_view* out) {
+  MHIMX_CHECK_ARG(out && R >= 1 && R <= 32768 && k >= 1 && k <= 6, "merge_ws_view_of: the projection-free form's workspace (1 <= R <= 32768, 1 <= k <= 6)");
+  int64_t o[3];
+  merge2_ws_view(R, k, o);
+  out->premul = o[0]; out->Y = o[1]; out->O = o[2];
+  return 0;
+}
 extern "C" int64_t mhimx_merge_part_floats(void) { return merge2_part_floats(); }
 extern "C" int mhimx_merge_fwd_part(void* stream, const mhimx_merge* m, const float* X, int64_t R, float* part, void* ws, int64_t ws_bytes) {
   if (int r = check_merge(m)) return r;
diff --git a/mhim_mil_amd/csrc/mca2.hip b/mhim_mil_amd/csrc/mca2.hip
--- a/mhim_mil_amd/csrc/mca2.hip
+++ b/mhim_mil_amd/csrc/mca2.hip
@@ -6,6 +6,7 @@
 namespace mhimx {
 
 int64_t merge2_part_floats() { return M2_PART_FLOATS; }
+int64_t merge2_premul_floats() { return M2_PREMUL_FLOATS; }
 int64_t merge2_rows_tiles(int64_t R) { return cdiv(R, m2_tile_rows(R)); }
 int64_t merge2_ws_bytes(int64_t R, int64_t k) {
   Arena ar(nullptr, 0);
@@ -20,7 +21,8 @@
 
 __global__ __launch_bounds__(M2_THREADS) void merge2_prep_kernel(Merge2PrepArgs a) {
   __shared__ __attribute__((aligned(16))) float lds[6 * M2_E + 6 * 64];
-  merge2_prep_body((int)blockIdx.x, lds, a.q_param, a.ln_w, a.ln_b, a.wq, a.wkv, a.k, a.scale, a.w);
+  if (blockIdx.x < M2_PREP_BLOCKS) merge2_prep_body((int)blockIdx.x, lds, a.q_param, a.ln_w, a.ln_b, a.wq, a.wkv, a.k, a.scale, a.w);
+  else merge2_premul_body((int)blockIdx.x - M2_PREP_BLOCKS, (int)gridDim.x - M2_PREP_BLOCKS, a.wo, a.wkv, a.w.Mw);
 }
 
 template <int RT>
@@ -48,11 +50,9 @@
   merge2_partials_body<MODE>((int)blockIdx.x, lds, in, live_only != 0, ln_w, ln_b, out, stats, raw_stats);
 }
 
-__global__ __launch_bounds__(M2_THREADS) void merge2_o_kernel(const float* __restrict__ wkv, int k, Merge2Ws w, BagBatch bb) {
-  __shared__ __attribute__((aligned(16))) float ys[6 * M2_E];
-  bag_move(w, bb);
+MHIMX_DEV void merge2_o_body(int block, float* ys , const float* __restrict__ wkv, int k, const Merge2Ws& w) {
   const int tid = threadIdx.x;
-  const int h = blockIdx.x >> 2, qd = blockIdx.x & 3;
+  const int h = block >> 2, qd = block & 3;
   M2HeadRows wr;
   m2_head_rows_load<16>(wkv + (int64_t)(M2_I + h * 64 + qd * 16) * M2_E, wr);
   m2_zero_tail(ys, k);
@@ -60,6 +60,79 @@
     reinterpret_cast<m2_f4*>(ys)[idx] = reinterpret_cast<const m2_f4*>(w.Y + (int64_t)h * k * M2_E)[idx];
   __syncthreads();
   m2_head_dots_use<16>(wr, ys, k, nullptr, 16, w.O + h * 64 + qd * 16);
+}
+__global__ __launch_bounds__(M2_THREADS) void merge2_o_kernel(const float* __restrict__ wkv, int k, Merge2Ws w, BagBatch bb) {
+  __shared__ __attribute__((aligned(16))) float ys[6 * M2_E];
+  bag_move(w, bb);
+  merge2_o_body((int)blockIdx.x, ys, wkv, k, w);
+}
+
+constexpr int M2_OUT_COLS = 2, M2_OUT_BLOCKS = M2_E / M2_OUT_COLS, M2_O_BLOCKS = M2_H * 4;
+__global__ __launch_bounds__(M2_THREADS) void merge2_out_kernel(const float* __restrict__ wkv, const float* __restrict__ bo, int k, float p, uint64_t seed0,
+                                                               const uint64_t* __restrict__ tick, float* __restrict__ z, const float* q, float* q_new,
+                                                               float mm, Merge2Ws w, BagBatch bb) {
+  __shared__ __attribute__((aligned(16))) float ys[6 * M2_E];
+  __shared__ float part[4][M2_OUT_COLS][8];
+  if (blockIdx.z) {
+    MHIMX_BAG(z); MHIMX_BAG(q); MHIMX_BAG(q_new);
+    seed0 = bag_mca_seed(seed0, bb);
+    bag_move(w, bb);
+  }
+  if (blockIdx.x >= M2_OUT_BLOCKS) {
+    merge2_o_body((int)blockIdx.x - M2_OUT_BLOCKS, ys, wkv, k, w);
+    return;
+  }
+  const int tid = threadIdx.x, lane = tid & 63, wave = tid >> 6;
+  const int n0 = blockIdx.x * M2_OUT_COLS;
+  const int ec = (tid >> 3) & (M2_OUT_COLS - 1), ei = tid & 7;
+  const bool fin = tid < M2_OUT_COLS * 8 && ei < k;
+  const uint64_t seed = p > 0.f ? eff_seed(seed0, tick) : 0;
+  const float bias = fin ? bo[n0 + ec] : 0.f;
+  const float qv = (fin && q_new) ? q[(int64_t)ei * M2_E + n0 + ec] : 0.f;
+  m2_f4 mv[2][2][M2_OUT_COLS], yv[2][2][6];
+#pragma unroll
+  for (int hh = 0; hh < 2; ++hh) {
+    const int h = 2 * wave + hh;
+#pragma unroll
+    for (int half = 0; half < 2; ++half) {
+      const int c = half * 256 + 4 * lane;
+#pragma unroll
+      for (int cc = 0; cc < M2_OUT_COLS; ++cc)
+        mv[hh][half][cc] = *reinterpret_cast<const m2_f4*>(w.Mw + ((int64_t)h * M2_E + n0 + cc) * M2_E + c);
+#pragma unroll
+      for (int i = 0; i < 6; ++i)
+        yv[hh][half][i] = *reinterpret_cast<const m2_f4*>(w.Y + (int64_t)(h * k + (i < k ? i : k - 1)) * M2_E + c);
+    }
+  }
+  float acc[M2_OUT_COLS][6];
+#pragma unroll
+  for (int cc = 0; cc < M2_OUT_COLS; ++cc)
+#pragma unroll
+    for (int i = 0; i < 6; ++i) acc[cc][i] = 0.f;
+#pragma unroll
+  for (int hh = 0; hh < 2; ++hh)
+#pragma unroll
+    for (int half = 0; half < 2; ++half)
+#pragma unroll
+      for (int u = 0; u < 4; ++u)
+#pragma unroll
+        for (int cc = 0; cc < M2_OUT_COLS; ++cc)
+#pragma unroll
+          for (int i = 0; i < 6; ++i) acc[cc][i] = __builtin_fmaf(mv[hh][half][cc][u], yv[hh][half][i][u], acc[cc][i]);
+#pragma unroll
+  for (int cc = 0; cc < M2_OUT_COLS; ++cc)
+#pragma unroll
+    for (int i = 0; i < 6; ++i)
+      if (i < k) {
+        const float s = wave_sum(acc[cc][i]);
+        if (lane == 0) part[wave][cc][i] = s;
+      }
+  __syncthreads();
+  if (!fin) return;
+  float v = ((part[0][ec][ei] + part[1][ec][ei]) + part[2][ec][ei]) + part[3][ec][ei] + bias;
+  if (p > 0.f) v = drop_keep(seed, (uint64_t)ei, (uint32_t)(n0 + ec), p) ? v * (1.f / (1.f - p)) : 0.f;
+  z[(int64_t)ei * M2_E + n0 + ec] = v;
+  if (q_new) q_new[(int64_t)ei * M2_E + n0 + ec] = qv * mm + v * (1.f - mm);
 }
 
 __global__ __launch_bounds__(M2_THREADS) void merge2_bwd_pre_kernel(const float* __restrict__ dz, const float* __restrict__ wo_t,
@@ -150,7 +223,8 @@
     return 0;
   }
   if (!m->prepared) {
-    hipLaunchKernelGGL(merge2_prep_kernel, dim3(64), dim3(M2_THREADS), 0, st, Merge2PrepArgs{m->q_param, m->ln_w, m->ln_b, m->wq, m->wkv, k, scale, w});
+    hipLaunchKernelGGL(merge2_prep_kernel, dim3(M2_PREP_BLOCKS + M2_PREMUL_ITEMS), dim3(M2_THREADS), 0, st,
+                       Merge2PrepArgs{m->q_param, m->ln_w, m->ln_b, m->wq, m->wkv, m->wo, k, scale, w});
     MHIMX_LAUNCH_CHECK();
   }
   MHIMX_ONCE_PER_DEVICE(MHIMX_HIP(hipFuncSetAttribute((const void*)merge2_rows_fwd_kernel<32>, hipFuncAttributeMaxDynamicSharedMemorySize, (int)m2_fwd_smem(32)));
@@ -165,15 +239,28 @@
   *wout = w;
   return 0;
 }
-static int merge2_fwd_tail(hipStream_t st, const mhimx_merge* m, float* z, float* q_new, int update_q, const Merge2Ws& w) {
+static int merge2_fwd_tail(hipStream_t st, const mhimx_merge* m, float* z, float* q_new, int update_q, const Merge2Ws& w, int two_launch) {
   const int k = (int)m->k;
-  hipLaunchKernelGGL(merge2_o_kernel, bgrid(M2_H * 4), dim3(M2_THREADS), 0, st, m->wkv, k, w, cur_batch());
-  MHIMX_LAUNCH_CHECK();
-  return mca_out(st, w.O, m->wo, m->bo, k, M2_E, M2_I, m->drop_p, m->drop_seed + 0x9E3779B97F4A7C15ull, m->drop_tick, z, m->q_param,
-                 update_q ? q_new : (float*)nullptr, m->mm);
-}
-
-int merge2_fwd(hipStream_t st, const mhimx_merge* m, const float* X, int64_t R, float* z, float* q_new, int update_q, void* ws, int64_t ws_bytes) {
+  const uint64_t oseed = m->drop_seed + 0x9E3779B97F4A7C15ull;
+  if (!two_launch) {
+    hipLaunchKernelGGL(merge2_out_kernel, bgrid(M2_OUT_BLOCKS + M2_O_BLOCKS), dim3(M2_THREADS), 0, st, m->wkv, m->bo, k, m->drop_p, oseed, m->drop_tick, z,
+                       m->q_param, update_q ? q_new : (float*)nullptr, m->mm, w, cur_batch());
+    MHIMX_LAUNCH_CHECK();
+    return 0;
+  }
+  hipLaunchKernelGGL(merge2_o_kernel, bgrid(M2_O_BLOCKS), dim3(M2_THREADS), 0, st, m->wkv, k, w, cur_batch());
+  MHIMX_LAUNCH_CHECK();
+  return mca_out(st, w.O, m->wo, m->bo, k, M2_E, M2_I, m->drop_p, oseed, m->drop_tick, z, m->q_param, update_q ? q_new : (float*)nullptr, m->mm);
+}
+void merge2_ws_view(int64_t R, int64_t k, int64_t* out) {
+  Arena ar(nullptr, 0);
+  Merge2Ws w;
+  merge2_ws_layout(ar, R, k, &w);
+  out[0] = (int64_t)reinterpret_cast<intptr_t>(w.Mw); out[1] = (int64_t)reinterpret_cast<intptr_t>(w.Y); out[2] = (int64_t)reinterpret_cast<intptr_t>(w.O);
+}
+
+int merge2_fwd(hipStream_t st, const mhimx_merge* m, const float* X, int64_t R, float* z, float* q_new, int update_q, void* ws, int64_t ws_bytes,
+               int two_launch) {
   MHIMX_CHECK_ARG(!update_q || q_new, "merge_fwd: update_q needs q_new");
   MHIMX_CHECK_ARG(m->own_n == 0, "merge_fwd: a shard of an instance-sharded bag runs mhimx_merge_fwd_part + mhimx_merge_fwd_finish");
   Merge2Ws w;
@@ -182,7 +269,7 @@
   hipLaunchKernelGGL(merge2_partials_kernel<1>, bgrid((unsigned)(J * 4)), dim3(M2_THREADS), 0, st, m2_parts_tiles(w, w.ypart), 0, m->ln_w, m->ln_b, w.Y,
                      w.stats, (float*)nullptr, cur_batch());
   MHIMX_LAUNCH_CHECK();
-  return merge2_fwd_tail(st, m, z, q_new, update_q, w);
+  return merge2_fwd_tail(st, m, z, q_new, update_q, w, two_launch);
 }
 
 int merge2_fwd_part(hipStream_t st, const mhimx_merge* m, const float* X, int64_t R, float* part, void* ws, int64_t ws_bytes) {
@@ -207,7 +294,7 @@
   hipLaunchKernelGGL(merge2_partials_kernel<1>, dim3((unsigned)(J * 4)), dim3(M2_THREADS), 0, st, m2_parts_shards(parts, W), 0, m->ln_w, m->ln_b, w.Y,
                      w.stats, (float*)nullptr, BagBatch{});
   MHIMX_LAUNCH_CHECK();
-  return merge2_fwd_tail(st, m, z, q_new, update_q, w);
+  return merge2_fwd_tail(st, m, z, q_new, update_q, w, 0);
 }
 
 int gemm_tn_rider(hipStream_t st, const mhimx_gemm_tn_args& g, const Merge2Side* rider, int stage);
@@ -305,7 +392,8 @@
   Merge2Ws w;
   merge2_ws_layout(ar, R, m->k, &w);
   MHIMX_CHECK_ARG(ar.ok(), "prep_batch: Merge workspace too small (%lld < %lld)", (long long)ws_bytes, (long long)ar.off);
-  *out = Merge2PrepArgs{m->q_param, m->ln_w, m->ln_b, m->wq, m->wkv, (int)m->k, 1.0f / sqrtf((float)M2_DH), w};
-  return 0;
-}
-}
+  MHIMX_CHECK_ARG(m->wo && aligned16(m->wo), "prep_batch: the Merge preparation job reads to_out's weight (16-byte aligned)");
+  *out = Merge2PrepArgs{m->q_param, m->ln_w, m->ln_b, m->wq, m->wkv, m->wo, (int)m->k, 1.0f / sqrtf((float)M2_DH), w};
+  return 0;
+}
+}
diff --git a/mhim_mil_amd/csrc/mca2_prep.hpp b/mhim_mil_amd/csrc/mca2_prep.hpp
--- a/mhim_mil_amd/csrc/mca2_prep.hpp
+++ b/mhim_mil_amd/csrc/mca2_prep.hpp
@@ -8,10 +8,14 @@
 constexpr int M2_XLD = M2_E + 4;
 constexpr int M2_PLD = 36;
 constexpr int M2_CLD = 2 * M2_JK + 4;
+constexpr int M2_PREP_BLOCKS = 64;
+constexpr int M2_PREMUL_ITEMS = 256;
+constexpr int64_t M2_PREMUL_FLOATS = (int64_t)M2_H * M2_E * M2_E;
 
 typedef float m2_f4 __attribute__((ext_vector_type(4)));
 
 struct Merge2Ws {
+  float* Mw;
   float *gq, *gmean, *grstd, *Q, *aq, *aqf, *gtf_aq, *mean, *rstd, *S, *pm, *pl, *psd, *ypart, *stats, *Y, *O;
   float *dO, *dyf, *gtf_dy, *dpart, *upart, *lnpart, *dQ;
   unsigned* gate;
@@ -38,6 +42,7 @@
   w.rt = m2_tile_rows(R);
   const int64_t T = cdiv(R, w.rt);
   w.T = (int)T;
+  w.Mw = cur_premul() ? cur_premul() : ar.take<float>(M2_PREMUL_FLOATS);
   w.gq = ar.take<float>(k * M2_E);
   w.gmean = ar.take<float>(k);
   w.grstd = ar.take<float>(k);
@@ -203,7 +208,31 @@
     if ((tid >> 6) == ((j - J) >> 3) % 4) m2_store_images(w.aqf, w.gtf_aq, j, e, 0.f);
 }
 
-
-struct Merge2PrepArgs { const float *q_param, *ln_w, *ln_b, *wq, *wkv; int k; float scale; Merge2Ws w; };
-
-}
+MHIMX_DEV void merge2_premul_body(int block, int nblk, const float* __restrict__ wo, const float* __restrict__ wkv, float* __restrict__ Mw) {
+  const int tid = threadIdx.x;
+  for (int item = block; item < M2_PREMUL_ITEMS; item += nblk) {
+    const int h = item >> 5, n0 = (item & 31) * 16;
+    const float* wv = wkv + (int64_t)(M2_I + h * M2_DH) * M2_E + tid;
+    const float* wr = wo + (int64_t)n0 * M2_I + h * M2_DH;
+    float a0[16], a1[16];
+#pragma unroll
+    for (int r = 0; r < 16; ++r) { a0[r] = 0.f; a1[r] = 0.f; }
+#pragma unroll 8
+    for (int d = 0; d < M2_DH; ++d) {
+      const float v0 = wv[(int64_t)d * M2_E], v1 = wv[(int64_t)d * M2_E + 256];
+#pragma unroll
+      for (int r = 0; r < 16; ++r) {
+        const float c = wr[(int64_t)r * M2_I + d];
+        a0[r] = __builtin_fmaf(c, v0, a0[r]);
+        a1[r] = __builtin_fmaf(c, v1, a1[r]);
+      }
+    }
+    float* out = Mw + ((int64_t)h * M2_E + n0) * M2_E + tid;
+#pragma unroll
+    for (int r = 0; r < 16; ++r) { out[(int64_t)r * M2_E] = a0[r]; out[(int64_t)r * M2_E + 256] = a1[r]; }
+  }
+}
+
+struct Merge2PrepArgs { const float *q_param, *ln_w, *ln_b, *wq, *wkv, *wo; int k; float scale; Merge2Ws w; };
+
+}
diff --git a/mhim_mil_amd/csrc/prep_jobs.hpp b/mhim_mil_amd/csrc/prep_jobs.hpp
--- a/mhim_mil_amd/csrc/prep_jobs.hpp
+++ b/mhim_mil_amd/csrc/prep_jobs.hpp
@@ -147,7 +147,9 @@
     Merge2Ws w = pj.m2.w;
     const int64_t sh = pj.m2_shift[jb.R];
     w.gq += sh; w.gmean += sh; w.grstd += sh; w.Q += sh; w.aq += sh; w.aqf += sh; w.gtf_aq += sh; w.gate += sh;
-    merge2_prep_body(bid, lds, pj.m2.q_param, pj.m2.ln_w, pj.m2.ln_b, pj.m2.wq, pj.m2.wkv, pj.m2.k, pj.m2.scale, w);
+    w.Mw += sh;
+    if (bid < M2_PREP_BLOCKS) merge2_prep_body(bid, lds, pj.m2.q_param, pj.m2.ln_w, pj.m2.ln_b, pj.m2.wq, pj.m2.wkv, pj.m2.k, pj.m2.scale, w);
+    else merge2_premul_body(bid - M2_PREP_BLOCKS, nblk - M2_PREP_BLOCKS, pj.m2.wo, pj.m2.wkv, w.Mw);
   }
 }
 
diff --git a/mhim_mil_amd/csrc/ragged_window.hip b/mhim_mil_amd/csrc/ragged_window.hip
--- a/mhim_mil_amd/csrc/ragged_window.hip
+++ b/mhim_mil_amd/csrc/ragged_window.hip
@@ -325,6 +325,8 @@
   const uint64_t* tick = c.tick;
 
   const mhimx_merge mw_prep = mid_merge_params(c);
+  mhimx_merge mw_prep_later = mw_prep;
+  mw_prep_later.prepared = 1;
   {
     mhimx_prep_job jobs[10];
     int n = mid_prep_head(c, im, jobs);
@@ -373,7 +375,7 @@
     {
       mhimx_prep_job jobs[2];
       jobs[0] = mhimx_prep_job{10, nullptr, reinterpret_cast<float*>(rows_all + g.cnt.len_keep), N, k};
-      jobs[1] = mhimx_prep_job{6, reinterpret_cast<const float*>(&mw_prep), static_cast<float*>(merge_ws), R, w.merge_ws_bytes};
+      jobs[1] = mhimx_prep_job{6, reinterpret_cast<const float*>(b == 0 ? &mw_prep : &mw_prep_later), static_cast<float*>(merge_ws), R, w.merge_ws_bytes};
       if (int r = mhimx_prep_batch(stream, jobs, 2)) return r;
     }
     const MidBag mb = {H_s + row0 * E, dHall + row0 * E, rows_all, N, R, g.cnt.Lk, g.seeds.mca, F(w.q_scr), F(w.s_s), F(w.stats_s), F(w.z_s) + (int64_t)b * E,
diff --git a/mhim_mil_amd/csrc/step.hip b/mhim_mil_amd/csrc/step.hip
--- a/mhim_mil_amd/csrc/step.hip
+++ b/mhim_mil_amd/csrc/step.hip
@@ -526,13 +526,16 @@
   const int64_t g_lo = E * D;
 
   const mhimx_merge mw_prep = mid_merge_params(c);
+  mhimx_merge mw_prep_later = mw_prep;
+  mw_prep_later.prepared = 1;
   {
     mhimx_prep_job jobs[MHIMX_PREP_MAX];
     int n = mid_prep_head(c, im, jobs);
     n += mid_prep_student(c, im, jobs + n);
     for (int i = 0; i < n_bags; ++i) {
       jobs[n++] = mhimx_prep_job{10, nullptr, reinterpret_cast<float*>(reinterpret_cast<int64_t*>(bag(b.rows_all, i)) + len_keep), N, k};
-      jobs[n++] = mhimx_prep_job{6, reinterpret_cast<const float*>(&mw_prep), reinterpret_cast<float*>(bag(b.merge_ws, i)), R, b.merge_ws_bytes};
+      jobs[n++] = mhimx_prep_job{6, reinterpret_cast<const float*>(i == 0 ? &mw_prep : &mw_prep_later), reinterpret_cast<float*>(bag(b.merge_ws, i)), R,
+                                 b.merge_ws_bytes};
     }
     static_assert(10 + 2 * MHIMX_WINDOW_MAX <= MHIMX_PREP_MAX, "the window's preparation is one launch");
     if (int r = mhimx_prep_batch(stream, jobs, n)) return r;
diff --git a/mhim_mil_amd/ops.py b/mhim_mil_amd/ops.py
--- a/mhim_mil_amd/ops.py
+++ b/mhim_mil_amd/ops.py
@@ -521,6 +521,24 @@
                                     ws.numel()), "mhimx_merge_fwd")
     mw.c.rows_done = 0
     return z, q_new, ws
+
+
+def merge_fwd_two_launch(mw: MergeW, X, update_q=True, ws=None):
+    _chk(X, name="X")
+    R = X.shape[0] if mw.x_rows is None else mw.x_rows.shape[0]
+    z = torch.empty((mw.k, mw.E), device=X.device)
+    q_new = torch.empty((mw.k, mw.E), device=X.device) if update_q else None
+    ws = ws if ws is not None else mw.ws_for(R, X.device)
+    L.check(L.lib().mhimx_merge_fwd_two_launch(_stream(), C.byref(mw.c), _p(X), R, _p(z), _p(q_new), int(bool(update_q)), _p(ws), ws.numel()),
+            "mhimx_merge_fwd_two_launch")
+    return z, q_new, ws
+
+
+def merge_ws_views(ws, R, k):
+    v = L.MergeWsView()
+    L.check(L.lib().mhimx_merge_ws_view_of(int(R), int(k), C.byref(v)), "mhimx_merge_ws_view_of")
+    f = lambda off, n: ws[off:off + 4 * n].view(torch.float32)
+    return f(v.premul, 8 * 512 * 512).view(8, 512, 512), f(v.Y, 8 * k * 512).view(8 * k, 512), f(v.O, k * 512).view(k, 512)
 
 
 def merge_fwd_part(mw: MergeW, X, ws=None, part=None):
```

New measurement: 32.65 million patch-instances/s. -2.9%, worse.
